# bearcove/loona

Hardware: AMD Instinct MI355X
Metric: Huffman header-literal decode GiB/s (device-resident) at 1/2/4/8 MI355X (higher is better)
Workload: dtype u8

## Files before the change

loona_amd/csrc/hpk_code.h:

```cpp
#pragma once
#include <stdint.h>

#define HPK_NSYM 257
#define HPK_EOS 256
#define HPK_LUT_BITS 12
#define HPK_LUT_SIZE (1u << HPK_LUT_BITS)
#define HPK_LO_RUNS 30
#define HPK_LO_SIZE (HPK_LO_RUNS * 32)

#define HPK_LIM5 0x50000000u
#define HPK_LIM6 0xB8000000u
#define HPK_LIM7 0xF8000000u
#define HPK_LIM8 0xFE000000u

static const uint8_t HPK_CODE_LEN[HPK_NSYM] = {
    13, 23, 28, 28, 28, 28, 28, 28, 28, 24, 30, 28, 28, 30, 28, 28,
    28, 28, 28, 28, 28, 28, 30, 28, 28, 28, 28, 28, 28, 28, 28, 28,
    6,  10, 10, 12, 13, 6,  8,  11, 10, 10, 8,  11, 8,  6,  6,  6,
    5,  5,  5,  6,  6,  6,  6,  6,  6,  6,  7,  8,  15, 6,  12, 10,
    13, 6,  7,  7,  7,  7,  7,  7,  7,  7,  7,  7,  7,  7,  7,  7,
    7,  7,  7,  7,  7,  7,  7,  7,  8,  7,  8,  13, 19, 13, 14, 6,
    15, 5,  6,  5,  6,  5,  6,  6,  6,  5,  7,  7,  6,  6,  6,  5,
    6,  7,  6,  5,  5,  6,  7,  7,  7,  7,  7,  15, 11, 14, 13, 28,
    20, 22, 20, 20, 22, 22, 22, 23, 22, 23, 23, 23, 23, 23, 24, 23,
    24, 24, 22, 23, 24, 23, 23, 23, 23, 21, 22, 23, 22, 23, 23, 24,
    22, 21, 20, 22, 22, 23, 23, 21, 23, 22, 22, 24, 21, 22, 23, 23,
    21, 21, 22, 21, 23, 22, 23, 23, 20, 22, 22, 22, 23, 22, 22, 23,
    26, 26, 20, 19, 22, 23, 22, 25, 26, 26, 26, 27, 27, 26, 24, 25,
    19, 21, 26, 27, 27, 26, 27, 24, 21, 21, 26, 26, 28, 27, 27, 27,
    20, 24, 20, 21, 22, 21, 21, 23, 22, 22, 25, 25, 24, 24, 26, 23,
    26, 27, 26, 26, 27, 27, 27, 27, 27, 28, 27, 27, 27, 27, 27, 26,
    30,
};

#define HPK_LUT2_NOTTWO 0x40000000u
#define HPK_LUT2_NONE 0x80000000u
#define HPK_LUT2_MISSING 15u
#define HPK_LUT2_CLAMP 14u
#define HPK_L2_LEN0(e) (((e) >> 8) & 15u)
#define HPK_L2_HELD(e) (((e) >> 12) & 15u)
#define HPK_L2_LEN01(e) (((e) >> 24) & 15u)
#define HPK_L2_CODES(e) (((e) >> 28) & 3u)
#define HPK_L2_TWO(e) (((e) >> 29) & 1u)

#define HPK_L3_HELD(e) (((e) >> 8) & 0xFFu)
#define HPK_L3_CODES(e) (((e) >> 24) & 3u)
#define HPK_L3_LEN0(e) (((e) >> 26) & 15u)
#define HPK_L3_NOTTWO 0x80000000u

struct hpk_tables {
    uint32_t code[HPK_NSYM];
    uint8_t len[HPK_NSYM];
    uint32_t lut[HPK_LUT_SIZE];
    uint32_t lut2[HPK_LUT_SIZE];
    uint32_t lut3[HPK_LUT_SIZE];
    uint16_t lo[HPK_LO_SIZE];
    uint8_t t8[256];
};

static inline int hpk_build_tables(hpk_tables* t) {
    uint16_t order[HPK_NSYM];
    int n = 0;
    for (int L = 1; L <= 30; ++L)
        for (int s = 0; s < HPK_NSYM; ++s)
            if (HPK_CODE_LEN[s] == L) order[n++] = (uint16_t)s;
    if (n != HPK_NSYM) return -1;
    uint64_t c = 0;
    int prev = HPK_CODE_LEN[order[0]];
    for (int i = 0; i < n; ++i) {
        int s = order[i], L = HPK_CODE_LEN[s];
        if (i) c = (c + 1) << (L - prev);
        prev = L;
        t->code[s] = (uint32_t)c;
        t->len[s] = (uint8_t)L;
    }
    if (c + 1 != (1ull << prev)) return -1;

    for (int k = 0; k < HPK_LO_RUNS; ++k)
        for (int t5 = 0; t5 < 32; ++t5) {
            uint64_t w = ((((1ull << k) - 1) << 6) | (uint64_t)t5) << (64 - (k + 6));
            uint16_t e = 0xFFFF;
            for (int s = 0; s < HPK_NSYM; ++s) {
                int L = t->len[s];
                if ((w >> (64 - L)) == t->code[s]) { e = (uint16_t)(s | (L << 9)); break; }
            }
            if (e == 0xFFFF) return -1;
            t->lo[k * 32 + t5] = e;
        }

    for (uint32_t v = 0; v < 256; ++v) {
        t->t8[v] = 0;
        const uint32_t w = v << 24;
        if (w >= HPK_LIM8) continue;
        const int L = 5 + (w >= HPK_LIM5) + (w >= HPK_LIM6) + (w >= HPK_LIM7);
        int found = -1;
        for (int s = 0; s < 256; ++s)
            if (t->len[s] <= 8 && (w >> (32 - t->len[s])) == t->code[s]) { found = s; break; }
        if (found < 0 || t->len[found] != L) return -1;
        t->t8[v] = (uint8_t)found;
    }

    for (uint32_t v = 0; v < HPK_LUT_SIZE; ++v) {
        uint32_t w = v << (32 - HPK_LUT_BITS);
        int s0 = -1, l0 = 0;
        for (int s = 0; s < 256; ++s) {
            int L = t->len[s];
            if (L <= HPK_LUT_BITS && (w >> (32 - L)) == t->code[s]) { s0 = s; l0 = L; break; }
        }
        if (s0 < 0) {
            t->lut[v] = 0;
            t->lut2[v] = 0xC0000000u | (HPK_LUT2_MISSING << 8) | (HPK_LUT2_MISSING << 24);
            continue;
        }
        uint32_t w1 = w << l0;
        int rem = HPK_LUT_BITS - l0, s1 = -1, l1 = 0;
        for (int s = 0; s < 256 && rem >= 5; ++s) {
            int L = t->len[s];
            if (L <= rem && (w1 >> (32 - L)) == t->code[s]) { s1 = s; l1 = L; break; }
        }
        uint32_t e = (uint32_t)s0 | ((uint32_t)l0 << 16);
        uint32_t e2 = (uint32_t)s0 | ((uint32_t)l0 << 8);
        if (s1 >= 0) {
            e |= ((uint32_t)s1 << 8) | ((uint32_t)(l0 + l1) << 21) | (2u << 26);
            e2 |= ((uint32_t)s1 << 16) | ((uint32_t)(l0 + l1) << 24) | ((uint32_t)(l0 + l1) << 12) | (2u << 28);
        } else {
            e |= ((uint32_t)l0 << 21) | (1u << 26);
            e2 |= (HPK_LUT2_MISSING << 24) | ((uint32_t)l0 << 12) | (1u << 28) | HPK_LUT2_NOTTWO;
        }
        t->lut[v] = e;
        t->lut2[v] = e2;
    }
    for (uint32_t v = 0; v < HPK_LUT_SIZE; ++v) {
        const uint32_t e2 = t->lut2[v], codes = HPK_L2_CODES(e2);
        t->lut3[v] = (e2 & 0xFFu) | (HPK_L2_HELD(e2) << 8) | (e2 & 0x00FF0000u) | (codes << 24) |
                     ((codes ? HPK_L2_LEN0(e2) : 15u) << 26) | (codes < 2 ? HPK_L3_NOTTWO : 0u);
    }
    return 0;
}
```

loona_amd/csrc/hpk_ctx.hip:

```cpp
#include <stdio.h>
#include <string.h>
#include <sys/mman.h>

#include <initializer_list>

#include "hpk_device.h"

#define HPK_VERSION "hpk 0.38 gfx950 decode v38 (every batch: wave fills, each wave with its own LDS window and image, longest-first queue, slot end offsets by DPP, nontemporal window loads stopping at the chunk's last byte, nontemporal write-back; chunks by guided self-scheduling from 4M literals, fixed 96-literal chunks below; fills and long-literal phase: body steps with no fit tests while >= 29 bits are left, then the wave fills' tails as four masked lookups with no fit test per code (checked steps only for a 13..28-bit code or a cut code in the tail) and the other kernels' checked tails (the long phase's at its refill points); long literals one lane each streaming from HBM after the fills, dense ranges listed longest-first; literals of >= 8 KiB by a whole workgroup in speculative pieces; compacted-output form: wave fills packed per workgroup from an LDS cursor into a bound layout made from the input offsets, each lane storing its two literals in unaligned 16-byte pieces; small-call mode: a persistent kernel behind a host-mapped doorbell); encode v5 (byte-balanced workgroup ranges, start map and DPP segmented scan, run accumulator, LDS image, live chunks only)"

static thread_local std::string t_last_error;

int hpk_set_err(const char* what, hipError_t e) {
    char buf[256];
    snprintf(buf, sizeof buf, "%s: %s", what, hipGetErrorString(e));
    t_last_error = buf;
    return HPK_E_DEVICE;
}

int hpk_set_err_msg(const char* what, int code) {
    t_last_error = what;
    return code;
}


extern "C" const char* hpk_version(void) { return HPK_VERSION; }

extern "C" const char* hpk_last_error(const hpk_ctx*) { return t_last_error.c_str(); }

extern "C" hpk_ctx* hpk_ctx_create(int device) {
    const hpk_tables* t = hpk_get_tables();
    if (!t) { hpk_set_err_msg("code table build failed", HPK_E_INVAL); return nullptr; }
    int ndev = 0;
    hipError_t e = hipGetDeviceCount(&ndev);
    if (e != hipSuccess || ndev <= 0) { hpk_set_err("hipGetDeviceCount", e); return nullptr; }
    if (device < 0 || device >= ndev) { hpk_set_err_msg("device index out of range", HPK_E_INVAL); return nullptr; }
    hpk_ctx* c = new hpk_ctx();
    c->device = device;
    auto fail = [&](const char* what, hipError_t err) {
        hpk_set_err(what, err);
        hpk_ctx_destroy(c);
        return (hpk_ctx*)nullptr;
    };
    if ((e = hipSetDevice(device)) != hipSuccess) return fail("hipSetDevice", e);
    hipDeviceProp_t prop;
    if ((e = hipGetDeviceProperties(&prop, device)) != hipSuccess) return fail("hipGetDeviceProperties", e);
    if (strncmp(prop.gcnArchName, "gfx950", 6) != 0) {
        hpk_set_err_msg("libhpk kernels are built for gfx950 only", HPK_E_NODEVICE);
        delete c;
        return nullptr;
    }
    c->num_cu = prop.multiProcessorCount;
    if ((e = hipStreamCreateWithFlags(&c->own, hipStreamNonBlocking)) != hipSuccess) return fail("hipStreamCreate", e);
    c->stream = c->own;
    if ((e = hipMalloc(&c->d_lut, sizeof(t->lut))) != hipSuccess) return fail("hipMalloc lut", e);
    if ((e = hipMemcpy(c->d_lut, t->lut, sizeof(t->lut), hipMemcpyHostToDevice)) != hipSuccess) return fail("upload lut", e);
    if ((e = hipMalloc(&c->d_lut2, sizeof(t->lut2))) != hipSuccess) return fail("hipMalloc lut2", e);
    if ((e = hipMemcpy(c->d_lut2, t->lut2, sizeof(t->lut2), hipMemcpyHostToDevice)) != hipSuccess)
        return fail("upload lut2", e);
    if ((e = hipMalloc(&c->d_lut3, sizeof(t->lut3))) != hipSuccess) return fail("hipMalloc lut3", e);
    if ((e = hipMemcpy(c->d_lut3, t->lut3, sizeof(t->lut3), hipMemcpyHostToDevice)) != hipSuccess)
        return fail("upload lut3", e);
    if ((e = hipMalloc(&c->d_lo, sizeof(t->lo))) != hipSuccess) return fail("hipMalloc lo", e);
    if ((e = hipMalloc(&c->d_t8, sizeof(t->t8))) != hipSuccess) return fail("hipMalloc t8", e);
    if ((e = hipMemcpy(c->d_t8, t->t8, sizeof(t->t8), hipMemcpyHostToDevice)) != hipSuccess) return fail("upload t8", e);
    if ((e = hipMalloc(&c->d_codes, 2 * 257 * sizeof(uint32_t))) != hipSuccess) return fail("hipMalloc codes", e);
    uint32_t packed[2 * 257];
    for (int s = 0; s < 257; ++s) {
        packed[s] = t->code[s];
        packed[257 + s] = t->len[s];
    }
    if ((e = hipMemcpy(c->d_lo, t->lo, sizeof(t->lo), hipMemcpyHostToDevice)) != hipSuccess) return fail("upload lo", e);
    if ((e = hipMemcpy(c->d_codes, packed, sizeof(packed), hipMemcpyHostToDevice)) != hipSuccess) return fail("upload codes", e);
    if ((e = hipHostMalloc((void**)&c->h_err, 64, hipHostMallocMapped | hipHostMallocCoherent)) != hipSuccess)
        return fail("hipHostMalloc err flag", e);
    *c->h_err = 0;
    if ((e = hipHostGetDevicePointer((void**)&c->d_err, c->h_err, 0)) != hipSuccess) return fail("err flag pointer", e);
    return c;
}

static int grow(void** p, size_t* cap, size_t need) {
    if (need <= *cap) return HPK_E_OK;
    size_t n = need + need / 4 + 4096;
    (void)hipFree(*p);
    *p = nullptr;
    *cap = 0;
    HIP_TRY(hipMalloc(p, n));
    *cap = n;
    return HPK_E_OK;
}

static int slot_acquire(hpk_ctx* c, hpk_slot** slot) {
    hpk_slot* s = nullptr;
    bool any = false;
    for (hpk_slot& k : c->slots) {
        if (k.used && k.stream == c->stream) s = &k;
        any |= k.used;
    }
    if (!s) {
        if (any && !c->slot_events) {
            c->slot_events = true;
            HIP_TRY(hipStreamSynchronize(c->own));
            for (hpk_slot& k : c->slots)
                if (k.stream == c->own) k.ev_set = false;
        }
        int j = 0;
        while (j < hpk_ctx::kSlots && c->slots[j].used) ++j;
        if (j == hpk_ctx::kSlots) {
            j = c->slot_next;
            c->slot_next = (j + 1) % hpk_ctx::kSlots;
            if (c->slots[j].ev_set) HIP_TRY(hipEventSynchronize(c->slots[j].ev));
        }
        s = &c->slots[j];
        s->stream = c->stream;
    }
    if (c->slot_events && !s->ev) HIP_TRY(hipEventCreateWithFlags(&s->ev, hipEventDisableTiming));
    *slot = s;
    return HPK_E_OK;
}

struct slot_need {
    DevBuf* buf;
    size_t bytes;
};
static int slot_reserve(hpk_ctx* c, hpk_slot* s, std::initializer_list<slot_need> needs) {
    bool small = false;
    for (const slot_need& nd : needs) small |= nd.buf->cap < nd.bytes;
    if (small) {
        if (s->ev_set)
            HIP_TRY(hipEventSynchronize(s->ev));
        else if (s->used)
            HIP_TRY(hipStreamSynchronize(c->own));
        for (const slot_need& nd : needs)
            if (int rc = grow(&nd.buf->p, &nd.buf->cap, nd.bytes)) return rc;
    }
    s->used = true;
    return HPK_E_OK;
}

static int slot_commit(hpk_ctx* c, hpk_slot* s) {
    if (!c->slot_events && c->stream == c->own) return HPK_E_OK;
    if (!s->ev) HIP_TRY(hipEventCreateWithFlags(&s->ev, hipEventDisableTiming));
    HIP_TRY(hipEventRecord(s->ev, c->stream));
    s->ev_set = true;
    return HPK_E_OK;
}

extern "C" void hpk_ctx_destroy(hpk_ctx* c) {
    if (!c) return;
    (void)hipSetDevice(c->device);
    (void)hpk_persist_stop(c);
    if (c->sm_stream) (void)hipStreamDestroy(c->sm_stream);
    if (c->h_sm) (void)hipHostFree(c->h_sm);
    (void)hipFree(c->d_sm_dev);
    (void)hipStreamSynchronize(c->stream);
    (void)hipFree(c->d_lut);
    (void)hipFree(c->d_lut2);
    (void)hipFree(c->d_lut3);
    (void)hipFree(c->d_lo);
    (void)hipFree(c->d_t8);
    (void)hipFree(c->d_codes);
    (void)hipFree(c->d_in);
    (void)hipFree(c->d_out);
    (void)hipFree(c->d_meta);
    (void)hipFree(c->d_st);
    if (c->h_err) (void)hipHostFree(c->h_err);
    if (c->h_pin) (void)hipHostFree(c->h_pin);
    for (hpk_slot& s : c->slots) {
        if (s.ev_set) (void)hipEventSynchronize(s.ev);
        for (DevBuf* b : {&s.long_list, &s.cp_bound, &s.cp_tmp, &s.cp_cursor, &s.pk_scratch, &s.pk_bound, &s.pk_tmp})
            (void)hipFree(b->p);
        if (s.ev) (void)hipEventDestroy(s.ev);
    }
    for (int j = 0; j < hpk_ctx::kMaxChunks; ++j) {
        if (c->ev_in[j]) (void)hipEventDestroy(c->ev_in[j]);
        if (c->ev_run[j]) (void)hipEventDestroy(c->ev_run[j]);
        if (c->ev_out[j]) (void)hipEventDestroy(c->ev_out[j]);
    }
    if (c->h2d) (void)hipStreamDestroy(c->h2d);
    if (c->d2h) (void)hipStreamDestroy(c->d2h);
    if (c->own) (void)hipStreamDestroy(c->own);
    delete c;
}

extern "C" int hpk_ctx_set_stream(hpk_ctx* c, void* s) {
    if (!c) return HPK_E_INVAL;
    if (s == HPK_STREAM_LEGACY)
        c->stream = (hipStream_t)0;
    else
        c->stream = s ? (hipStream_t)s : c->own;
    return HPK_E_OK;
}

extern "C" int hpk_host_register(void* ptr, size_t bytes) {
    if (!ptr || !bytes) return hpk_set_err_msg("null range", HPK_E_INVAL);
    HIP_TRY(hipHostRegister(ptr, bytes, hipHostRegisterDefault));
    return HPK_E_OK;
}

extern "C" int hpk_host_unregister(void* ptr) {
    if (!ptr) return hpk_set_err_msg("null pointer", HPK_E_INVAL);
    HIP_TRY(hipHostUnregister(ptr));
    return HPK_E_OK;
}

int hpk_ctx_pinned(hpk_ctx* c, size_t bytes, void** p) {
    if (bytes > c->h_pin_cap) {
        HIP_TRY(hipSetDevice(c->device));
        HIP_TRY(hipStreamSynchronize(c->stream));
        if (c->d2h) HIP_TRY(hipStreamSynchronize(c->d2h));
        if (c->h_pin) (void)hipHostFree(c->h_pin);
        c->h_pin = nullptr;
        c->h_pin_cap = 0;
        const size_t cap = bytes + bytes / 4 + (1u << 20);
        HIP_TRY(hipHostMalloc(&c->h_pin, cap, hipHostMallocDefault));
        c->h_pin_cap = cap;
    }
    *p = c->h_pin;
    return HPK_E_OK;
}

extern "C" int hpk_ctx_set_decode_kernel(hpk_ctx* c, int kind) {
    if (!c || kind < HPK_DECODE_AUTO || kind > HPK_DECODE_WAVE) return hpk_set_err_msg("bad decode kernel", HPK_E_INVAL);
    c->decode_kernel = kind;
    return HPK_E_OK;
}

extern "C" void* hpk_ctx_stream(hpk_ctx* c) { return c ? (void*)c->stream : nullptr; }

extern "C" int hpk_ctx_set_small_mode(hpk_ctx* c, uint32_t max_literals, int workgroups, uint32_t idle_ms) {
    if (!c) return HPK_E_INVAL;
    HIP_TRY(hipSetDevice(c->device));
    if (max_literals == 0) {
        const int rc = hpk_persist_stop(c);
        c->sm_max = 0;
        return rc;
    }
    if (workgroups < 1 || workgroups > 16 || workgroups >= c->num_cu || idle_ms < 1 || idle_ms > 10000 ||
        max_literals > (uint32_t)workgroups * 256u * 64u)
        return hpk_set_err_msg("small mode: 1-16 workgroups, 1-10000 ms idle, at most 64 literals per lane", HPK_E_INVAL);
    if (!c->h_sm) {
        HIP_TRY(hipStreamCreateWithFlags(&c->sm_stream, hipStreamNonBlocking));
        HIP_TRY(hipHostMalloc(&c->h_sm, 256, hipHostMallocMapped | hipHostMallocCoherent));
        memset(c->h_sm, 0, 256);
        HIP_TRY(hipHostGetDevicePointer(&c->d_sm, c->h_sm, 0));
        HIP_TRY(hipMalloc(&c->d_sm_dev, 128));
    }
    if (c->sm_launched && (workgroups != c->sm_wgs || idle_ms != c->sm_idle_ms))
        if (int rc = hpk_persist_stop(c)) return rc;
    c->sm_max = max_literals;
    c->sm_wgs = workgroups;
    c->sm_idle_ms = idle_ms;
    return c->sm_launched ? HPK_E_OK : hpk_persist_start(c);
}

extern "C" int hpk_ctx_sync(hpk_ctx* c) {
    if (!c) return HPK_E_INVAL;
    HIP_TRY(hipStreamSynchronize(c->stream));
    return HPK_E_OK;
}

static int check_offsets(const uint32_t* off, uint32_t n, size_t cap) {
    for (uint32_t i = 0; i < n; ++i)
        if (off[i + 1] < off[i]) return hpk_set_err_msg("offsets must be non-decreasing", HPK_E_INVAL);
    if (off[n] > cap || off[n] > HPK_MAX_OFFSET) return hpk_set_err_msg("offsets pass the blob's capacity", HPK_E_INVAL);
    return HPK_E_OK;
}

static int take_err(hpk_ctx* c) {
    if (!__atomic_exchange_n(c->h_err, 0u, __ATOMIC_ACQ_REL)) return HPK_E_OK;
    return hpk_set_err_msg("a batch had non-monotone offsets or offsets past a blob's capacity (HPK_BAD_OFFSETS)",
                           HPK_E_INVAL);
}

extern "C" int hpk_ctx_check(hpk_ctx* c) {
    if (!c) return HPK_E_INVAL;
    HIP_TRY(hipStreamSynchronize(c->stream));
    return take_err(c);
}

static int call_end(hpk_ctx* c, int flags) {
    if (flags & HPK_ASYNC) return HPK_E_OK;
    HIP_TRY(hipStreamSynchronize(c->stream));
    return take_err(c);
}

typedef int (*launch_fn)(hpk_ctx*, const hpk_batch&);

static int decode_region(hpk_ctx* c, const hpk_batch& b) {
    hpk_slot* s;
    int rc;
    if ((rc = slot_acquire(c, &s)) || (rc = slot_reserve(c, s, {{&s->long_list, 4 * (size_t)b.n}}))) return rc;
    if ((rc = hpk_launch_decode(c, b, s->long_list.as<uint32_t>()))) return rc;
    return slot_commit(c, s);
}

static uint32_t clamp_cap(size_t cap) { return cap > HPK_MAX_OFFSET ? HPK_MAX_OFFSET : (uint32_t)cap; }

static int queue_chunks(launch_fn fn, hpk_ctx* c, const uint8_t* in_blob, const uint32_t* in_off, uint8_t* out_blob,
                        const uint32_t* out_off, uint32_t* out_len, uint8_t* status, uint32_t n, size_t in_bytes,
                        size_t out_bytes, int chunks, const uint32_t* cut, uint32_t* d_in_off, uint32_t* d_out_off,
                        uint32_t* d_len);

static int host_begin(launch_fn fn, hpk_ctx* c, const uint8_t* in_blob, size_t in_cap, const uint32_t* in_off,
                      uint32_t n, uint8_t* out_blob, size_t out_cap, const uint32_t* out_off, uint32_t* out_len,
                      uint8_t* status, bool trusted, int* nchunks, uint32_t* cut) {
    *nchunks = 0;
    if (!trusted && (check_offsets(in_off, n, in_cap) || check_offsets(out_off, n, out_cap))) return HPK_E_INVAL;
    if (n == 0) return HPK_E_OK;
    const size_t in_bytes = in_off[n], out_bytes = out_off[n];
    if ((in_bytes && !in_blob) || (out_bytes && !out_blob)) return hpk_set_err_msg("null blob", HPK_E_INVAL);
    int rc;
    if ((rc = grow((void**)&c->d_in, &c->d_in_cap, in_bytes + 16))) return rc;
    if ((rc = grow((void**)&c->d_out, &c->d_out_cap, out_bytes + 16))) return rc;
    if ((rc = grow((void**)&c->d_meta, &c->d_meta_cap, (3 * (size_t)n + 2) * 4))) return rc;
    if ((rc = grow((void**)&c->d_st, &c->d_st_cap, n))) return rc;
    uint32_t* d_in_off = c->d_meta;
    uint32_t* d_out_off = c->d_meta + (n + 1);
    uint32_t* d_len = c->d_meta + 2 * ((size_t)n + 1);
    if (!c->h2d) {
        HIP_TRY(hipStreamCreateWithFlags(&c->h2d, hipStreamNonBlocking));
        HIP_TRY(hipStreamCreateWithFlags(&c->d2h, hipStreamNonBlocking));
        for (int j = 0; j < hpk_ctx::kMaxChunks; ++j) {
            HIP_TRY(hipEventCreateWithFlags(&c->ev_in[j], hipEventDisableTiming));
            HIP_TRY(hipEventCreateWithFlags(&c->ev_run[j], hipEventDisableTiming));
            HIP_TRY(hipEventCreateWithFlags(&c->ev_out[j], hipEventDisableTiming));
        }
    }
    const size_t kChunkBytes = (size_t)4 << 20;
    int chunks = (int)((in_bytes + out_bytes) / kChunkBytes);
    chunks = chunks < 1 ? 1 : (chunks > hpk_ctx::kMaxChunks ? hpk_ctx::kMaxChunks : chunks);
    if ((uint32_t)chunks > n) chunks = (int)n;
    cut[0] = 0;
    for (int j = 1; j < chunks; ++j) {
        const uint64_t target = (uint64_t)in_bytes * j / chunks;
        uint32_t lo = cut[j - 1], hi = n;
        while (lo < hi) {
            const uint32_t mid = lo + (hi - lo) / 2;
            if (in_off[mid + 1] < target) lo = mid + 1; else hi = mid;
        }
        cut[j] = lo;
    }
    cut[chunks] = n;
    auto drain = [&](int rc) {
        (void)hipStreamSynchronize(c->h2d);
        (void)hipStreamSynchronize(c->stream);
        (void)hipStreamSynchronize(c->d2h);
        return rc;
    };
    if (int e = queue_chunks(fn, c, in_blob, in_off, out_blob, out_off, out_len, status, n, in_bytes, out_bytes,
                             chunks, cut, d_in_off, d_out_off, d_len))
        return drain(e);
    *nchunks = chunks;
    return HPK_E_OK;
}

static int queue_chunks(launch_fn fn, hpk_ctx* c, const uint8_t* in_blob, const uint32_t* in_off, uint8_t* out_blob,
                        const uint32_t* out_off, uint32_t* out_len, uint8_t* status, uint32_t n, size_t in_bytes,
                        size_t out_bytes, int chunks, const uint32_t* cut, uint32_t* d_in_off, uint32_t* d_out_off,
                        uint32_t* d_len) {
    int rc;
    HIP_TRY(hipEventRecord(c->ev_run[0], c->stream));
    HIP_TRY(hipStreamWaitEvent(c->h2d, c->ev_run[0], 0));
    for (int j = 0; j < chunks; ++j) {
        const uint32_t a = cut[j], b = cut[j + 1];
        if (a < b) {
            const size_t ib = in_off[a], ie = in_off[b], ob = out_off[a], oe = out_off[b];
            if (ie > ib) HIP_TRY(hipMemcpyAsync(c->d_in + ib, in_blob + ib, ie - ib, hipMemcpyHostToDevice, c->h2d));
            HIP_TRY(hipMemcpyAsync(d_in_off + a, in_off + a, (b - a + 1) * 4ull, hipMemcpyHostToDevice, c->h2d));
            HIP_TRY(hipMemcpyAsync(d_out_off + a, out_off + a, (b - a + 1) * 4ull, hipMemcpyHostToDevice, c->h2d));
            HIP_TRY(hipEventRecord(c->ev_in[j], c->h2d));
            HIP_TRY(hipStreamWaitEvent(c->stream, c->ev_in[j], 0));
            const hpk_batch bt{c->d_in, (uint32_t)in_bytes, d_in_off + a, b - a, c->d_out, (uint32_t)out_bytes,
                               d_out_off + a, d_len + a, c->d_st + a};
            if ((rc = fn(c, bt))) return rc;
            HIP_TRY(hipEventRecord(c->ev_run[j], c->stream));
            HIP_TRY(hipStreamWaitEvent(c->d2h, c->ev_run[j], 0));
            if (oe > ob) HIP_TRY(hipMemcpyAsync(out_blob + ob, c->d_out + ob, oe - ob, hipMemcpyDeviceToHost, c->d2h));
            HIP_TRY(hipMemcpyAsync(out_len + a, d_len + a, (b - a) * 4ull, hipMemcpyDeviceToHost, c->d2h));
            HIP_TRY(hipMemcpyAsync(status + a, c->d_st + a, b - a, hipMemcpyDeviceToHost, c->d2h));
        }
        HIP_TRY(hipEventRecord(c->ev_out[j], c->d2h));
    }
    return HPK_E_OK;
}

static int host_end(hpk_ctx* c) {
    HIP_TRY(hipStreamSynchronize(c->d2h));
    return take_err(c);
}

static int run_batch(launch_fn fn, hpk_ctx* c, const uint8_t* in_blob, size_t in_cap, const uint32_t* in_off,
                     uint32_t n, uint8_t* out_blob, size_t out_cap, const uint32_t* out_off, uint32_t* out_len,
                     uint8_t* status, int flags) {
    if (!c || !in_off || !out_off || (n && (!out_len || !status))) return hpk_set_err_msg("null argument", HPK_E_INVAL);
    HIP_TRY(hipSetDevice(c->device));
    if (flags & HPK_PTR_DEVICE) {
        if (n == 0) return HPK_E_OK;
        if (!in_blob || !out_blob) return hpk_set_err_msg("null blob", HPK_E_INVAL);
        const hpk_batch b{in_blob, clamp_cap(in_cap), in_off, n, out_blob, clamp_cap(out_cap), out_off, out_len, status};
        if (fn == decode_region && !(flags & HPK_ASYNC) && c->sm_max) {
            bool handled = false;
            if (int rc = hpk_persist_call(c, b, &handled)) return rc;
            if (handled) return HPK_E_OK;
        }
        if (int rc = fn(c, b)) return rc;
        return call_end(c, flags);
    }
    int chunks;
    uint32_t cut[hpk_ctx::kMaxChunks + 1];
    if (int rc = host_begin(fn, c, in_blob, in_cap, in_off, n, out_blob, out_cap, out_off, out_len, status, false,
                            &chunks, cut))
        return rc;
    return chunks ? host_end(c) : HPK_E_OK;
}

int hpk_decode_host_begin(hpk_ctx* c, const uint8_t* in_blob, size_t in_cap, const uint32_t* in_off, uint32_t n,
                          uint8_t* out_blob, size_t out_cap, const uint32_t* out_off, uint32_t* out_len,
                          uint8_t* status, int* nchunks, uint32_t* cut) {
    HIP_TRY(hipSetDevice(c->device));
    return host_begin(decode_region, c, in_blob, in_cap, in_off, n, out_blob, out_cap, out_off, out_len, status,
                      true, nchunks, cut);
}

int hpk_host_chunk_wait(hpk_ctx* c, int j) {
    HIP_TRY(hipEventSynchronize(c->ev_out[j]));
    return HPK_E_OK;
}

int hpk_decode_host_end(hpk_ctx* c) { return host_end(c); }

int hpk_ctx_max_chunks() { return hpk_ctx::kMaxChunks; }

extern "C" int hpk_decode_batch(hpk_ctx* c, const uint8_t* in_blob, size_t in_cap, const uint32_t* in_off, uint32_t n,
                                uint8_t* out_blob, size_t out_cap, const uint32_t* out_off, uint32_t* out_len,
                                uint8_t* status, int flags) {
    return run_batch(decode_region, c, in_blob, in_cap, in_off, n, out_blob, out_cap, out_off, out_len, status,
                     flags);
}

static int check_call(const hpk_ctx* c, bool null_arg, int flags, uint32_t n, const char* what, const size_t* in_cap,
                      uint64_t* need) {
    auto inval = [&](const char* before, const char* after) {
        return hpk_set_err_msg((std::string(before) + what + after).c_str(), HPK_E_INVAL);
    };
    if (!c || null_arg) return hpk_set_err_msg("null argument", HPK_E_INVAL);
    if (!(flags & HPK_PTR_DEVICE)) return inval("the ", " takes device pointers only");
    if (n >= 0x7FFFFFFFu) return inval("too many literals for the ", "");
    if (in_cap) {
        *need = (uint64_t)hpk_decoded_bound(clamp_cap(*in_cap)) + 4ull * n;
        if (*need > HPK_MAX_OFFSET) return inval("the ", "'s output would pass 4 GiB");
    }
    return HPK_E_OK;
}

extern "C" int hpk_decode_batch_compact(hpk_ctx* c, const uint8_t* in_blob, size_t in_cap, const uint32_t* in_off,
                                        uint32_t n, uint8_t* out_blob, size_t out_cap, uint32_t* out_off,
                                        uint32_t* out_len, uint8_t* status, int flags) {
    uint64_t need;
    if (int rc = check_call(c, !in_off || !out_off || (n && (!out_len || !status)), flags, n, "compacted form", &in_cap,
                            &need))
        return rc;
    if (out_cap < need) return hpk_set_err_msg("out_cap below hpk_decoded_bound(in_cap) + 4 n", HPK_E_INVAL);
    HIP_TRY(hipSetDevice(c->device));
    if (n == 0) {
        HIP_TRY(hipMemsetAsync(out_off, 0, 4, c->stream));
        return call_end(c, flags);
    }
    if (!in_blob || !out_blob) return hpk_set_err_msg("null blob", HPK_E_INVAL);
    const bool wave = hpk_compact_wave(c, n);
    hpk_slot* s;
    int rc;
    if ((rc = slot_acquire(c, &s))) return rc;
    if (wave)
        rc = slot_reserve(c, s, {{&s->long_list, 4 * (size_t)n}});
    else
        rc = slot_reserve(c, s, {{&s->long_list, 4 * (size_t)n}, {&s->cp_bound, 4 * ((size_t)n + 1)},
                                 {&s->cp_tmp, hpk_bound_tmp_bytes(n)}, {&s->cp_cursor, 4}});
    if (rc) return rc;
    hpk_batch b{in_blob, clamp_cap(in_cap), in_off, n, out_blob, clamp_cap(out_cap), nullptr, out_len, status};
    uint32_t* cursor = nullptr;
    if (!wave) {
        b.out_off = s->cp_bound.as<uint32_t>();
        cursor = s->cp_cursor.as<uint32_t>();
        if ((rc = hpk_bound_scan(c, in_off, n, s->cp_bound.as<uint32_t>(), s->cp_tmp.p))) return rc;
        HIP_TRY(hipMemsetAsync(cursor, 0, 4, c->stream));
    }
    if ((rc = hpk_launch_decode_compact(c, b, out_off, s->long_list.as<uint32_t>(), cursor, wave))) return rc;
    if (!wave)
        HIP_TRY(hipMemcpyAsync(out_off + n, cursor, 4, hipMemcpyDeviceToDevice, c->stream));
    if ((rc = slot_commit(c, s))) return rc;
    return call_end(c, flags);
}

static int packed_end(hpk_ctx* c, const uint32_t* dst_off_n, size_t dst_cap, int flags) {
    if (flags & HPK_ASYNC) return HPK_E_OK;
    uint32_t total = 0;
    HIP_TRY(hipMemcpyAsync(&total, dst_off_n, 4, hipMemcpyDeviceToHost, c->stream));
    if (int rc = call_end(c, flags)) return rc;
    if ((size_t)total > dst_cap) return hpk_set_err_msg("the packed bytes pass the output capacity", HPK_E_NOSPACE);
    return HPK_E_OK;
}

extern "C" int hpk_decode_batch_packed(hpk_ctx* c, const uint8_t* in_blob, size_t in_cap, const uint32_t* in_off,
                                       uint32_t n, uint8_t* out_blob, size_t out_cap, uint32_t* out_off,
                                       uint32_t* out_len, uint8_t* status, int flags) {
    uint64_t need;
    if (int rc = check_call(c, !in_off || !out_off || (n && (!out_len || !status)), flags, n, "packed form", &in_cap, &need))
        return rc;
    if (n && (!in_blob || (!out_blob && out_cap))) return hpk_set_err_msg("null blob", HPK_E_INVAL);
    HIP_TRY(hipSetDevice(c->device));
    if (n == 0) {
        HIP_TRY(hipMemsetAsync(out_off, 0, 4, c->stream));
        return packed_end(c, out_off, out_cap, flags);
    }
    size_t tmp = hpk_bound_tmp_bytes(n);
    if (tmp < hpk_pack_tmp_bytes(n)) tmp = hpk_pack_tmp_bytes(n);
    hpk_slot* s;
    int rc;
    if ((rc = slot_acquire(c, &s)) ||
        (rc = slot_reserve(c, s, {{&s->long_list, 4 * (size_t)n}, {&s->pk_bound, 4 * ((size_t)n + 1)}, {&s->pk_tmp, tmp},
                                  {&s->pk_scratch, (size_t)need + 64}})))
        return rc;
    uint32_t* bound = s->pk_bound.as<uint32_t>();
    uint8_t* scratch = s->pk_scratch.as<uint8_t>();
    if ((rc = hpk_bound_scan(c, in_off, n, bound, s->pk_tmp.p))) return rc;
    const hpk_batch b{in_blob, clamp_cap(in_cap), in_off, n, scratch, (uint32_t)need, bound, out_len, status};
    if ((rc = hpk_launch_decode(c, b, s->long_list.as<uint32_t>()))) return rc;
    if ((rc = hpk_pack_launch(c, scratch, (uint32_t)need, bound, out_len, n, out_blob, clamp_cap(out_cap), out_off,
                              s->pk_tmp.p, need)))
        return rc;
    if ((rc = slot_commit(c, s))) return rc;
    return packed_end(c, out_off + n, out_cap, flags);
}

extern "C" int hpk_pack_batch(hpk_ctx* c, const uint8_t* src_blob, size_t src_cap, const uint32_t* src_off,
                              const uint32_t* src_len, uint32_t n, uint8_t* dst_blob, size_t dst_cap, uint32_t* dst_off,
                              int flags) {
    if (int rc = check_call(c, !dst_off || (n && (!src_off || !src_len)), flags, n, "pack", nullptr, nullptr)) return rc;
    if (n && ((!src_blob && src_cap) || (!dst_blob && dst_cap))) return hpk_set_err_msg("null blob", HPK_E_INVAL);
    HIP_TRY(hipSetDevice(c->device));
    hpk_slot* s;
    int rc;
    if ((rc = slot_acquire(c, &s)) || (rc = slot_reserve(c, s, {{&s->pk_tmp, hpk_pack_tmp_bytes(n)}}))) return rc;
    if ((rc = hpk_pack_launch(c, src_blob, clamp_cap(src_cap), src_off, src_len, n, dst_blob, clamp_cap(dst_cap), dst_off,
                              s->pk_tmp.p, HPK_MAX_OFFSET)))
        return rc;
    if ((rc = slot_commit(c, s))) return rc;
    return packed_end(c, dst_off + n, dst_cap, flags);
}

extern "C" int hpk_encode_batch(hpk_ctx* c, const uint8_t* in_blob, size_t in_cap, const uint32_t* in_off, uint32_t n,
                                uint8_t* out_blob, size_t out_cap, const uint32_t* out_off, uint32_t* out_len,
                                uint8_t* status, int flags) {
    return run_batch(hpk_launch_encode, c, in_blob, in_cap, in_off, n, out_blob, out_cap, out_off, out_len, status,
                     flags);
}

struct hpk_arena {
    void* base;
    size_t len;
    int pinned;
};

extern "C" hpk_arena* hpk_arena_create(size_t num_bufs, size_t buf_size, int pin) {
    if (!num_bufs || !buf_size || num_bufs > ((size_t)1 << 40) / buf_size) {
        hpk_set_err_msg("bad arena size", HPK_E_INVAL);
        return nullptr;
    }
    const size_t len = num_bufs * buf_size;
    void* p = mmap(nullptr, len, PROT_READ | PROT_WRITE, MAP_PRIVATE | MAP_ANONYMOUS, -1, 0);
    if (p == MAP_FAILED) {
        hpk_set_err_msg("mmap failed", HPK_E_INVAL);
        return nullptr;
    }
    hpk_arena* a = new hpk_arena{p, len, 0};
    if (pin) {
        const hipError_t e = hipHostRegister(p, len, hipHostRegisterDefault);
        if (e != hipSuccess) {
            hpk_set_err("hipHostRegister arena", e);
            munmap(p, len);
            delete a;
            return nullptr;
        }
        a->pinned = 1;
    }
    return a;
}

extern "C" void* hpk_arena_base(const hpk_arena* a) { return a ? a->base : nullptr; }
extern "C" size_t hpk_arena_len(const hpk_arena* a) { return a ? a->len : 0; }

extern "C" void hpk_arena_destroy(hpk_arena* a) {
    if (!a) return;
    if (a->pinned) (void)hipHostUnregister(a->base);
    munmap(a->base, a->len);
    delete a;
}
```

loona_amd/csrc/hpk_decode.hip:

```cpp
#include <stdlib.h>

#include <chrono>

#include "hpk_fill.h"
#include "hpk_wave.h"
#include "hpk_persist.h"

using namespace hpkdec;

constexpr int kWaves = 16, kW = 40960, kO = 79104, kQ = 2048, kRefillN = 2;
#ifndef HPK_LONG_MIN
#define HPK_LONG_MIN 64
#endif
#ifndef HPK_LONG_BIG
#define HPK_LONG_BIG 1024
#endif
using Geo = Geo12<kWaves, kW, kO, kQ>;
constexpr int kWaveWin = 3072, kWaveImg = 5888;
#ifndef HPK_WAVE_MIN
#define HPK_WAVE_MIN 0u
#endif
#ifndef HPK_WAVE_GUIDED
#define HPK_WAVE_GUIDED 1
#endif
#ifndef HPK_WAVE_RANK
#define HPK_WAVE_RANK 0
#endif
#ifndef HPK_WAVE_CHUNK
#define HPK_WAVE_CHUNK 224u
#endif
#define WAVE_KERNEL(m) hpk_decode_wave<m, kWaveWin, kWaveImg, HPK_WAVE_CHUNK, HPK_WAVE_GUIDED, HPK_WAVE_RANK>
#ifndef HPK_WAVE_GUIDED_MIN
#define HPK_WAVE_GUIDED_MIN 4000000u
#endif
#ifndef HPK_WAVE_SMALL_CHUNK
#define HPK_WAVE_SMALL_CHUNK 96u
#endif
#define WAVE_KERNEL_SMALL(m) hpk_decode_wave<m, kWaveWin, kWaveImg, HPK_WAVE_SMALL_CHUNK, 2, HPK_WAVE_RANK>
#define DEC_KERNEL(m) hpk_decode12<m, kWaves, kW, kO, kQ, kRefillN>

#ifdef HPK_DIAG
static int g_debug_mode = -1;
static unsigned long long* g_dbg = nullptr;
static size_t g_dbg_n = 0;

static int dbg_buffer(hpk_ctx* c, DecodeArgs& a, size_t need, bool zero) {
    if (need > g_dbg_n) {
        (void)hipFree(g_dbg);
        HIP_TRY(hipMalloc(&g_dbg, need * 8));
        g_dbg_n = need;
    }
    if (zero) HIP_TRY(hipMemsetAsync(g_dbg, 0, need * 8, c->stream));
    a.dbg = g_dbg;
    return HPK_E_OK;
}

extern "C" int hpk_debug_check(unsigned long long* host8) {
    return hipMemcpyFromSymbol(host8, HIP_SYMBOL(g_chk), 8 * sizeof(unsigned long long)) == hipSuccess ? 0 : -1;
}

extern "C" int hpk_debug_stamps(unsigned long long* host, size_t cap_entries) {
    if (!g_dbg) return 0;
    size_t n = g_dbg_n < cap_entries ? g_dbg_n : cap_entries;
    if (hipMemcpy(host, g_dbg, n * 8, hipMemcpyDeviceToHost) != hipSuccess) return -1;
    return (int)n;
}
#endif

static void decode_args(hpk_ctx* c, const hpk_batch& b, DecodeArgs& a) {
    const auto in = split16(b.in_blob);
    const auto out = split16(b.out_blob);
    a.in_base = in.base;
    a.in_mis = in.mis;
    a.in_off = b.in_off;
    a.n = b.n;
    a.out_base = out.base;
    a.out_mis = out.mis;
    a.out_off = b.out_off;
    a.out_len = b.out_len;
    a.status = b.status;
    a.t8 = c->d_t8;
    a.lo = c->d_lo;
    a.lut = c->d_lut;
    a.lut2 = c->d_lut2;
    a.lut3 = c->d_lut3;
    a.dbg = nullptr;
    a.in_cap = b.in_cap;
    a.out_cap = b.out_cap;
    a.err = c->d_err;
    a.lit_out = b.out_off;
    a.co_off = nullptr;
    a.cursor = nullptr;
}

static uint32_t decode_blocks(hpk_ctx* c, const hpk_batch& b) {
    uint64_t blocks = ((uint64_t)b.n + 63) / 64;
    if (blocks < ((uint64_t)b.in_cap + 32767) / 32768) blocks = ((uint64_t)b.in_cap + 32767) / 32768;
    if (blocks > (uint64_t)b.n) blocks = (uint64_t)b.n;
    const uint64_t cus = (uint64_t)c->num_cu - (c->sm_launched && c->sm_max ? (uint64_t)c->sm_wgs : 0u);
    if (blocks > cus) blocks = cus;
    if (blocks < 1) blocks = 1;
    return (uint32_t)blocks;
}

constexpr int kPersistThreads = 256;

static int persist_launch(hpk_ctx* c, uint32_t base) {
    auto* h = static_cast<PersistCtl*>(c->h_sm);
    if (c->sm_launched) HIP_TRY(hipStreamSynchronize(c->sm_stream));
    __atomic_store_n(&h->stop, 0u, __ATOMIC_RELAXED);
    __atomic_store_n(&h->done, base, __ATOMIC_RELAXED);
    __atomic_store_n(&h->declined, 0u, __ATOMIC_RELAXED);
    __atomic_store_n(&h->alive, 1u, __ATOMIC_RELEASE);
    const uint32_t init[4] = {0u, base, 0u, 0u};
    HIP_TRY(hipMemcpyAsync(c->d_sm_dev, init, sizeof init, hipMemcpyHostToDevice, c->sm_stream));
    PersistArgs a{static_cast<PersistCtl*>(c->d_sm), c->d_sm_dev, c->d_lut3, c->d_lo, base, c->sm_idle_ms * 100000u};
    hipLaunchKernelGGL(hpk_persist<kPersistThreads>, dim3((uint32_t)c->sm_wgs), dim3(kPersistThreads), 0, c->sm_stream, a);
    HIP_TRY(hipGetLastError());
    c->sm_launched = true;
    return HPK_E_OK;
}

int hpk_persist_start(hpk_ctx* c) { return persist_launch(c, c->sm_req); }

extern "C" uint64_t hpk_test_small_calls(const hpk_ctx* c) { return c ? c->sm_calls : 0u; }

extern "C" int hpk_test_small_stamps(const hpk_ctx* c, uint32_t* out10) {
    if (!c || !c->h_sm || !out10) return HPK_E_INVAL;
    const auto* h = static_cast<const PersistCtl*>(c->h_sm);
    for (int k = 0; k < 6; ++k) out10[k] = __atomic_load_n(&h->ts[k], __ATOMIC_ACQUIRE);
    for (int k = 0; k < 4; ++k) out10[6 + k] = __atomic_load_n(&h->tl[k], __ATOMIC_ACQUIRE);
    return HPK_E_OK;
}

int hpk_persist_stop(hpk_ctx* c) {
    if (!c->sm_launched) return HPK_E_OK;
    auto* h = static_cast<PersistCtl*>(c->h_sm);
    __atomic_store_n(&h->stop, 1u, __ATOMIC_RELEASE);
    HIP_TRY(hipStreamSynchronize(c->sm_stream));
    c->sm_launched = false;
    return HPK_E_OK;
}

int hpk_persist_call(hpk_ctx* c, const hpk_batch& b, bool* handled) {
    *handled = false;
    if (!c->sm_max || b.n > c->sm_max || b.n == 0) return HPK_E_OK;
    if (hipStreamQuery(c->stream) != hipSuccess) HIP_TRY(hipStreamSynchronize(c->stream));
    auto* h = static_cast<PersistCtl*>(c->h_sm);
    if (!c->sm_launched || __atomic_load_n(&h->alive, __ATOMIC_ACQUIRE) == 0u)
        if (int rc = persist_launch(c, c->sm_req)) return rc;
    const auto in = split16(b.in_blob);
    const auto out = split16(b.out_blob);
    h->in_base = in.base;
    h->out_base = out.base;
    h->in_off = b.in_off;
    h->out_off = b.out_off;
    h->out_len = b.out_len;
    h->status = b.status;
    h->n = b.n;
    h->in_mis = in.mis;
    h->out_mis = out.mis;
    h->in_cap = b.in_cap;
    h->out_cap = b.out_cap;
    const uint32_t k = ++c->sm_req;
    __atomic_store_n(&h->req, k, __ATOMIC_RELEASE);
    const auto t0 = std::chrono::steady_clock::now();
    for (uint32_t spins = 0; __atomic_load_n(&h->done, __ATOMIC_ACQUIRE) != k; ++spins) {
        if (__atomic_load_n(&h->alive, __ATOMIC_ACQUIRE) == 0u) {
            if (int rc = persist_launch(c, k - 1u)) return rc;
        }
        __builtin_ia32_pause();
        if ((spins & 4095u) == 4095u && std::chrono::steady_clock::now() - t0 > std::chrono::seconds(10))
            return hpk_set_err_msg("small-call mode: the persistent kernel did not answer", HPK_E_DEVICE);
    }
    *handled = __atomic_load_n(&h->declined, __ATOMIC_ACQUIRE) == 0u;
    c->sm_calls += *handled ? 1u : 0u;
    return HPK_E_OK;
}

bool hpk_compact_wave(const hpk_ctx* c, uint32_t n) {
    return c->decode_kernel == HPK_DECODE_WAVE || (c->decode_kernel == HPK_DECODE_AUTO && n >= HPK_WAVE_MIN);
}

int hpk_launch_decode_compact(hpk_ctx* c, const hpk_batch& b, uint32_t* co_off, uint32_t* long_list, uint32_t* cursor,
                              bool wave) {
    DecodeArgs a;
    decode_args(c, b, a);
    a.lit_out = co_off;
    a.co_off = co_off;
    a.cursor = cursor;
    a.long_list = long_list;
    a.long_min = HPK_LONG_MIN;
    a.long_big = HPK_LONG_BIG;
    if (wave) {
        a.cursor = nullptr;
        hipLaunchKernelGGL((hpk_decode_wave<0, kWaveWin, kWaveImg, HPK_WAVE_CHUNK, HPK_WAVE_GUIDED, HPK_WAVE_RANK, true>),
                           dim3(decode_blocks(c, b)), dim3(Geo::kBlock), 0, c->stream, a);
    } else {
        hipLaunchKernelGGL((hpk_decode12<0, kWaves, kW, kO, kQ, kRefillN, true>), dim3(decode_blocks(c, b)),
                           dim3(Geo::kBlock), 0, c->stream, a);
    }
    HIP_TRY(hipGetLastError());
    return HPK_E_OK;
}

int hpk_launch_decode(hpk_ctx* c, const hpk_batch& b, uint32_t* long_list) {
    DecodeArgs a;
    decode_args(c, b, a);
    a.long_list = long_list;
    a.long_min = HPK_LONG_MIN;
    a.long_big = HPK_LONG_BIG;
#ifdef HPK_DIAG
    if (const char* lm = getenv("HPK_LONG_MIN")) a.long_min = (uint32_t)atoi(lm);
    if (const char* lb = getenv("HPK_LONG_BIG")) a.long_big = (uint32_t)atoi(lb);
#endif
    const uint32_t blocks = decode_blocks(c, b);
    const dim3 grid(blocks), block(Geo::kBlock);
    bool wave = c->decode_kernel == HPK_DECODE_WAVE || (c->decode_kernel == HPK_DECODE_AUTO && b.n >= HPK_WAVE_MIN);
#ifdef HPK_DIAG
    if (const char* wk = getenv("HPK_DECODE_KERNEL")) wave = wk[0] == 'w';
    if (g_debug_mode < 0) {
        const char* dm = getenv("HPK_DEBUG_MODE");
        g_debug_mode = dm ? atoi(dm) : 0;
    }
    static const int wave_var = getenv("HPK_WAVE_VARIANT") ? atoi(getenv("HPK_WAVE_VARIANT")) : -1;
    if (wave && wave_var >= 0 && g_debug_mode == 0) {
        switch (wave_var) {
            case 0: hipLaunchKernelGGL((hpk_decode_wave<0, kWaveWin, kWaveImg, 224u, false, 0>), grid, block, 0, c->stream, a); break;
            case 1: hipLaunchKernelGGL((hpk_decode_wave<0, kWaveWin, kWaveImg, 224u, false, 1>), grid, block, 0, c->stream, a); break;
            case 2: hipLaunchKernelGGL((hpk_decode_wave<0, kWaveWin, kWaveImg, 224u, false, 2>), grid, block, 0, c->stream, a); break;
            case 3: hipLaunchKernelGGL((hpk_decode_wave<0, kWaveWin, kWaveImg, 224u, true, 0>), grid, block, 0, c->stream, a); break;
            case 4: hipLaunchKernelGGL((hpk_decode_wave<0, kWaveWin, kWaveImg, 224u, true, 1>), grid, block, 0, c->stream, a); break;
            case 5: hipLaunchKernelGGL((hpk_decode_wave<0, kWaveWin, kWaveImg, 224u, true, 2>), grid, block, 0, c->stream, a); break;
            default: hipLaunchKernelGGL((WAVE_KERNEL(0)), grid, block, 0, c->stream, a); break;
        }
        HIP_TRY(hipGetLastError());
        return HPK_E_OK;
    }
    if (g_debug_mode == 3 || g_debug_mode == 5) {
        const size_t waves = g_debug_mode == 3 ? kWaves : HPK_LONG_WAVES;
        if (int rc = dbg_buffer(c, a, (size_t)blocks * waves * 16, g_debug_mode == 5)) return rc;
    }
#define WAVE_MODE(m)                                                                  \
    case m:                                                                           \
        if (b.n < HPK_WAVE_GUIDED_MIN)                                                \
            hipLaunchKernelGGL(WAVE_KERNEL_SMALL(m), grid, block, 0, c->stream, a);   \
        else                                                                          \
            hipLaunchKernelGGL(WAVE_KERNEL(m), grid, block, 0, c->stream, a);         \
        break;
#define FILL_MODE(m) \
    case m: hipLaunchKernelGGL(DEC_KERNEL(m), grid, block, 0, c->stream, a); break;
    if (wave) {
        switch (g_debug_mode) {
            WAVE_MODE(1) WAVE_MODE(2) WAVE_MODE(3) WAVE_MODE(5) WAVE_MODE(6) WAVE_MODE(8) WAVE_MODE(9) WAVE_MODE(10)
            default: WAVE_MODE(0)
        }
    } else {
        switch (g_debug_mode) {
            FILL_MODE(1) FILL_MODE(2) FILL_MODE(3) FILL_MODE(4) FILL_MODE(5)
            default: FILL_MODE(0)
        }
    }
#else
    if (wave && b.n < HPK_WAVE_GUIDED_MIN)
        hipLaunchKernelGGL(WAVE_KERNEL_SMALL(0), grid, block, 0, c->stream, a);
    else if (wave)
        hipLaunchKernelGGL(WAVE_KERNEL(0), grid, block, 0, c->stream, a);
    else
        hipLaunchKernelGGL(DEC_KERNEL(0), grid, block, 0, c->stream, a);
#endif
    HIP_TRY(hipGetLastError());
    return HPK_E_OK;
}
```

loona_amd/csrc/hpk_decode_kernel.h:

```cpp
#pragma once
#include <stdint.h>

#include "hpk_device.h"
#include "hpk_walk.h"

namespace hpkdec {

constexpr int kT8Bytes = 256;
constexpr int kLoBytes = HPK_LO_SIZE * 2;
constexpr int kTabBytes = ((kT8Bytes + kLoBytes + 15) / 16) * 16;

struct DecodeArgs {
    const uint8_t* in_base;
    uint32_t in_mis;
    const uint32_t* in_off;
    uint32_t n;
    uint8_t* out_base;
    uint32_t out_mis;
    const uint32_t* out_off;
    uint32_t* out_len;
    uint8_t* status;
    const uint8_t* t8;
    const uint16_t* lo;
    const uint32_t* lut;
    const uint32_t* lut2;
    const uint32_t* lut3;
    unsigned long long* dbg;
    uint32_t in_cap, out_cap;
    uint32_t* err;
    uint32_t* long_list;
    uint32_t long_min, long_big;
    const uint32_t* lit_out;
    uint32_t* co_off;
    uint32_t* cursor;
};

constexpr uint32_t kHugeMax = 16;

typedef uint32_t u32u __attribute__((aligned(1)));
typedef uint32_t u32x4u __attribute__((ext_vector_type(4), aligned(1)));

constexpr uint32_t kListed = 0xFFFFFFFFu;

constexpr uint32_t kQ7Byte = 0x80000000u;

__device__ __forceinline__ uint32_t lpt_bucket(uint32_t nbytes) {
    const uint32_t b = nbytes < 96u ? (nbytes >> 1) : min(63u, 48u + ((nbytes - 96u) >> 7));
    return 63u - b;
}

__device__ __forceinline__ void lds_barrier() { asm volatile("s_waitcnt lgkmcnt(0)\n\ts_barrier" ::: "memory"); }

}
```

loona_amd/csrc/hpk_device.h:

```cpp
#pragma once
#include <hip/hip_runtime.h>
#include <stdint.h>

#include <string>

#include "../../include/hpk.h"
#include "hpk_code.h"
#include "hpk_internal.h"

template <class T>
struct hpk_split16 {
    T* base;
    uint32_t mis;
};
template <class T>
inline hpk_split16<T> split16(T* p) {
    const uintptr_t u = (uintptr_t)p;
    return {(T*)(u & ~(uintptr_t)15), (uint32_t)(u & 15)};
}

struct DevBuf {
    void* p = nullptr;
    size_t cap = 0;
    template <class T>
    T* as() const { return static_cast<T*>(p); }
};

struct hpk_slot {
    hipStream_t stream = nullptr;
    bool used = false;
    hipEvent_t ev = nullptr;
    bool ev_set = false;
    DevBuf long_list;
    DevBuf cp_bound, cp_tmp, cp_cursor;
    DevBuf pk_scratch, pk_bound, pk_tmp;
};

struct hpk_ctx {
    int device = 0;
    int num_cu = 256;
    int decode_kernel = HPK_DECODE_AUTO;
    hipStream_t own = nullptr;
    hipStream_t stream = nullptr;
    uint32_t* d_lut = nullptr;
    uint32_t* d_lut2 = nullptr;
    uint32_t* d_lut3 = nullptr;
    uint16_t* d_lo = nullptr;
    uint8_t* d_t8 = nullptr;
    uint32_t* d_codes = nullptr;
    uint8_t* d_in = nullptr;
    size_t d_in_cap = 0;
    uint8_t* d_out = nullptr;
    size_t d_out_cap = 0;
    uint32_t* d_meta = nullptr;
    size_t d_meta_cap = 0;
    uint8_t* d_st = nullptr;
    size_t d_st_cap = 0;
    void* h_pin = nullptr;
    size_t h_pin_cap = 0;
    static constexpr int kMaxChunks = 8;
    hipStream_t h2d = nullptr;
    hipStream_t d2h = nullptr;
    hipEvent_t ev_in[kMaxChunks] = {};
    hipEvent_t ev_run[kMaxChunks] = {};
    hipEvent_t ev_out[kMaxChunks] = {};
    uint32_t* h_err = nullptr;
    uint32_t* d_err = nullptr;
    static constexpr int kSlots = 8;
    hpk_slot slots[kSlots];
    int slot_next = 0;
    bool slot_events = false;
    uint32_t sm_max = 0;
    int sm_wgs = 0;
    uint32_t sm_idle_ms = 0;
    hipStream_t sm_stream = nullptr;
    void* h_sm = nullptr;
    void* d_sm = nullptr;
    uint32_t* d_sm_dev = nullptr;
    uint32_t sm_req = 0;
    bool sm_launched = false;
    uint64_t sm_calls = 0;
};

int hpk_persist_call(hpk_ctx* c, const struct hpk_batch& b, bool* handled);
int hpk_persist_start(hpk_ctx* c);
int hpk_persist_stop(hpk_ctx* c);

struct hpk_batch {
    const uint8_t* in_blob;
    uint32_t in_cap;
    const uint32_t* in_off;
    uint32_t n;
    uint8_t* out_blob;
    uint32_t out_cap;
    const uint32_t* out_off;
    uint32_t* out_len;
    uint8_t* status;
};

int hpk_set_err(const char* what, hipError_t e);
int hpk_set_err_msg(const char* what, int code);

#define HIP_TRY(call)                                            \
    do {                                                         \
        hipError_t _e = (call);                                  \
        if (_e != hipSuccess) return hpk_set_err(#call, _e);     \
    } while (0)

int hpk_launch_decode(hpk_ctx* c, const hpk_batch& b, uint32_t* long_list);
bool hpk_compact_wave(const hpk_ctx* c, uint32_t n);
int hpk_launch_decode_compact(hpk_ctx* c, const hpk_batch& b, uint32_t* co_off, uint32_t* long_list, uint32_t* cursor,
                              bool wave);
int hpk_launch_encode(hpk_ctx* c, const hpk_batch& b);
size_t hpk_bound_tmp_bytes(uint32_t n);
int hpk_bound_scan(hpk_ctx* c, const uint32_t* in_off, uint32_t n, uint32_t* out, void* tmp);
size_t hpk_pack_tmp_bytes(uint32_t n);
int hpk_pack_launch(hpk_ctx* c, const uint8_t* src_blob, uint32_t src_cap, const uint32_t* src_off, const uint32_t* src_len,
                    uint32_t n, uint8_t* dst_blob, uint32_t dst_cap, uint32_t* dst_off, void* tmp, uint64_t total_bound);

__device__ __forceinline__ uint32_t hpk_bswap32(uint32_t x) { return __builtin_bswap32(x); }
```

loona_amd/csrc/hpk_huge_piece.h:

```cpp
#pragma once
#include "hpk_walk.h"

namespace hpkdec {

#ifndef HPK_HUGE_MIN
#define HPK_HUGE_MIN 8192u
#endif
constexpr uint32_t kHugePieceMin = 64;
constexpr uint32_t kHugeTerm = 0x100u;
constexpr uint32_t kHugeNone = 0xFFFFFFFFu;
constexpr uint32_t kHugeLimit = 1u << 28;

struct HugeWalk {
    uint64_t win;
    uint32_t nb;
    uint32_t qi;
    uint32_t pos;
    uint4 c0, c1;
};

__device__ __forceinline__ uint32_t huge_sel(const uint4& c, uint32_t j) {
    const uint32_t sh = (j & 1u) * 32u;
    const uint32_t lo = (uint32_t)((((uint64_t)c.y << 32) | c.x) >> sh);
    const uint32_t hi = (uint32_t)((((uint64_t)c.w << 32) | c.z) >> sh);
    return (j & 2u) ? hi : lo;
}

template <class Ld>
__device__ __forceinline__ void huge_begin(HugeWalk& W, const Ld& ld16, uint32_t lbyte, uint32_t pos) {
    const uint32_t b = lbyte + (pos >> 3);
    const uint32_t qd = b >> 2;
    const uint32_t sk = (b & 3u) * 8u + (pos & 7u);
    W.c0 = ld16(qd >> 2);
    W.c1 = ld16((qd >> 2) + 1u);
    W.win = ((uint64_t)__builtin_bswap32(huge_sel(W.c0, qd & 3u)) << 32) << sk;
    W.nb = 32u - sk;
    W.qi = qd + 1u;
    W.pos = pos;
    if ((W.qi & 3u) == 0u) {
        W.c0 = W.c1;
        W.c1 = ld16((W.qi >> 2) + 1u);
    }
}

template <int kTab, class Ld>
__device__ __forceinline__ void huge_peek(HugeWalk& W, const Ld& ld16, const uint32_t* __restrict__ lut,
                                          const uint16_t* __restrict__ lo, uint32_t& sym, uint32_t& len, bool& eos,
                                          uint32_t& sym1, uint32_t& held) {
    if (W.nb <= 32u) {
        W.win |= (uint64_t)__builtin_bswap32(huge_sel(W.c0, W.qi & 3u)) << (32u - W.nb);
        W.nb += 32u;
        W.qi += 1u;
        if ((W.qi & 3u) == 0u) {
            W.c0 = W.c1;
            W.c1 = ld16((W.qi >> 2) + 1u);
        }
    }
    const uint32_t w = (uint32_t)(W.win >> 32);
    const uint32_t e = lut[w >> (32 - HPK_LUT_BITS)];
    const uint32_t l0 = kTab == 3 ? HPK_L3_LEN0(e) : HPK_L2_LEN0(e);
    if (l0 <= (uint32_t)HPK_LUT_BITS) {
        sym = e & 0xFFu;
        len = l0;
        eos = false;
        const uint32_t codes = kTab == 3 ? HPK_L3_CODES(e) : HPK_L2_CODES(e);
        held = codes == 2u ? (kTab == 3 ? HPK_L3_HELD(e) : HPK_L2_HELD(e)) : 0u;
        sym1 = (e >> 16) & 0xFFu;
    } else {
        lo_decode(w, lo, sym, len, eos);
        held = 0;
        sym1 = 0;
    }
}

__device__ __forceinline__ void huge_adv(HugeWalk& W, uint32_t len) {
    W.win <<= len;
    W.nb -= len;
    W.pos += len;
}

template <int kTab, class Ld>
__device__ __forceinline__ uint32_t huge_count(HugeWalk& W, const Ld& ld16, const uint32_t* __restrict__ lut,
                                               const uint16_t* __restrict__ lo, uint32_t nbits, uint32_t nx, bool last,
                                               uint32_t& c) {
    c = 0;
    for (;;) {
        if (!last && W.pos >= nx) return 0u;
        uint32_t sym, len, sym1, held;
        bool eos;
        huge_peek<kTab>(W, ld16, lut, lo, sym, len, eos, sym1, held);
        const uint32_t rem = nbits - W.pos;
        if (held != 0u && held <= rem && (last || W.pos + len < nx)) {
            huge_adv(W, held);
            c += 2u;
            continue;
        }
        if (len > rem) return kHugeTerm | residual_status(rem, (uint32_t)(W.win >> 32));
        if (eos) return kHugeTerm | HPK_EOS_IN_STRING;
        huge_adv(W, len);
        c += 1u;
    }
}

__device__ __forceinline__ void huge_geometry(uint32_t nbytes, uint32_t lanes, uint32_t& P, uint32_t& PB, uint32_t& OV) {
    P = min(lanes, (nbytes + kHugePieceMin - 1u) / kHugePieceMin);
    PB = (nbytes + P - 1u) / P;
    P = (nbytes + PB - 1u) / PB;
    OV = PB >= 512u ? 512u : 256u;
}

template <int kTab, class Ld>
__device__ __forceinline__ void huge_pass1(const Ld& ld16, const uint32_t* __restrict__ lut, const uint16_t* __restrict__ lo,
                                           uint32_t lbyte, uint32_t nbytes, uint32_t k, uint32_t P, uint32_t PB,
                                           uint32_t OV, uint32_t& S, uint32_t& E, uint32_t& c, uint32_t& fl) {
    const uint32_t nbits = nbytes * 8u, st = k * PB * 8u;
    const bool last = k + 1u == P;
    const uint32_t nx = last ? nbits : (k + 1u) * PB * 8u;
    HugeWalk W;
    huge_begin(W, ld16, lbyte, k == 0u ? 0u : (st > OV ? st - OV : 0u));
    c = 0;
    fl = 0;
    while (W.pos < st) {
        uint32_t sym, len, sym1, held;
        bool eos;
        huge_peek<kTab>(W, ld16, lut, lo, sym, len, eos, sym1, held);
        if (held != 0u && held <= nbits - W.pos && W.pos + len < st) {
            huge_adv(W, held);
            continue;
        }
        if (len > nbits - W.pos || eos) {
            S = E = kHugeNone;
            return;
        }
        huge_adv(W, len);
    }
    S = W.pos;
    fl = huge_count<kTab>(W, ld16, lut, lo, nbits, nx, last, c);
    E = W.pos;
}

template <int kTab, class Ld>
__device__ __forceinline__ void huge_refix(const Ld& ld16, const uint32_t* __restrict__ lut, const uint16_t* __restrict__ lo,
                                           uint32_t lbyte, uint32_t nbytes, uint32_t k, uint32_t P, uint32_t PB,
                                           uint32_t from, uint32_t& S, uint32_t& E, uint32_t& c, uint32_t& fl) {
    const uint32_t nbits = nbytes * 8u;
    const bool last = k + 1u == P;
    const uint32_t nx = last ? nbits : (k + 1u) * PB * 8u;
    HugeWalk W;
    huge_begin(W, ld16, lbyte, from);
    S = from;
    fl = huge_count<kTab>(W, ld16, lut, lo, nbits, nx, last, c);
    E = W.pos;
}

template <int kTab, class Ld, class St8, class St1>
__device__ __forceinline__ void huge_pass2(const Ld& ld16, const uint32_t* __restrict__ lut, const uint16_t* __restrict__ lo,
                                           uint32_t lbyte, uint32_t S, uint32_t c, uint32_t ob, const St8& st8,
                                           const St1& st1) {
    HugeWalk W;
    huge_begin(W, ld16, lbyte, S);
    uint64_t acc = 0;
    uint32_t p = ob;
    auto emit = [&](uint32_t sym) {
        acc |= (uint64_t)sym << (8u * (p & 7u));
        if ((p & 7u) == 7u) {
            const uint32_t g = p - 7u;
            if (g >= ob) {
                st8(g, acc);
            } else {
                for (uint32_t x = ob; x <= p; ++x) st1(x, (uint8_t)(acc >> (8u * (x & 7u))));
            }
            acc = 0;
        }
        p += 1u;
    };
    for (uint32_t j = 0; j < c;) {
        uint32_t sym, len, sym1, held;
        bool eos;
        huge_peek<kTab>(W, ld16, lut, lo, sym, len, eos, sym1, held);
        emit(sym);
        if (held != 0u && j + 2u <= c) {
            emit(sym1);
            huge_adv(W, held);
            j += 2u;
        } else {
            huge_adv(W, len);
            j += 1u;
        }
    }
    for (uint32_t x = max(ob, p & ~7u); x < p; ++x) st1(x, (uint8_t)(acc >> (8u * (x & 7u))));
}

}
```

loona_amd/csrc/hpk_long.h:

```cpp
#pragma once
#include "hpk_decode_kernel.h"

namespace hpkdec {

typedef uint32_t u32x4 __attribute__((ext_vector_type(4)));

__device__ __forceinline__ __amdgpu_buffer_rsrc_t buf_rsrc(const void* p, uint32_t bytes) {
    return __builtin_amdgcn_make_buffer_rsrc(const_cast<void*>(p), 0, (int)bytes, 0x00020000);
}

__device__ __forceinline__ void store_part(__amdgpu_buffer_rsrc_t r, uint32_t gb, uint32_t lo, uint32_t hi,
                                           const uint32_t (&v)[4], const uint32_t (&b)[16]) {
#pragma unroll
    for (uint32_t d = 0; d < 4u; ++d) {
        if (lo <= 4u * d && 4u * d + 4u <= hi) {
            __builtin_amdgcn_raw_buffer_store_b32(v[d], r, gb, 4 * d, 0);
        } else {
#pragma unroll
            for (uint32_t e = 0; e < 4u; ++e)
                if (4u * d + e >= lo && 4u * d + e < hi)
                    __builtin_amdgcn_raw_buffer_store_b8((uint8_t)b[4u * d + e], r, gb, 4 * d + e, 0);
        }
    }
}

__device__ __forceinline__ uint32_t lpt_class_of(uint32_t nb);

__device__ __forceinline__ void pin(uint32_t x) { asm volatile("" ::"v"(x)); }

#ifndef HPK_LONG_WAVES
#define HPK_LONG_WAVES 8
#endif
#ifndef HPK_LONG_U
#define HPK_LONG_U 8
#endif
#ifndef HPK_LONG_CLAIM
#define HPK_LONG_CLAIM 64
#endif
#ifndef HPK_LONG_RING
#define HPK_LONG_RING 32
#endif

#ifndef HPK_LONG_TAILPT
#define HPK_LONG_TAILPT 1
#endif

#ifndef HPK_LONG_CH
#define HPK_LONG_CH 3
#endif

#ifndef HPK_LONG_OS
#define HPK_LONG_OS 80
#endif

#ifndef HPK_LONG_BODY
#define HPK_LONG_BODY 1
#endif

__device__ __forceinline__ uint32_t lpt_class_of(uint32_t nb) { return 31u - min(nb >> 7, 31u); }

template <int kBlock, int kU, int kRing, int kDiag, int kBlockAll, int kOSz = HPK_LONG_OS, int kClaim = 64,
          int kTab = 2,
          bool kCompact = false,
          int kCh = HPK_LONG_CH>
__device__ __forceinline__ void long_phase(const DecodeArgs& a, uint32_t ba, uint32_t bb, uint32_t c1, uint32_t c2,
                                           uint32_t* s_claim, uint32_t* s_ring, uint8_t* s_out, uint4* s_q,
                                           const uint32_t* s_lut, const uint16_t* s_lo) {
    constexpr uint32_t kChunk = kClaim;
    constexpr uint32_t kQ = kChunk;
    static_assert(kClaim == 32 || kClaim == 64, "claim size");
    constexpr uint32_t kOS = kOSz;
    static_assert(15 + 5 * kU + 3 + (HPK_LONG_TAILPT ? 6 : 0) < (int)kOS, "output buffer");
    static_assert((kRing & (kRing - 1)) == 0 && kRing >= 16 && 4 * kCh + 8 <= kRing, "input ring: a power of two >= 16 dwords");
    static_assert(kBlock % 64 == 0 && kBlock <= kBlockAll, "decoding waves");
    const uint32_t tid = threadIdx.x, lane = tid & 63u, wv = tid >> 6;
    const uint32_t total = c1 + c2;
    if (total == 0) return;
    if (tid >= (uint32_t)kBlock) return;
    uint4 (*sq)[kQ] = reinterpret_cast<uint4 (*)[kQ]>(s_q);
    const uint32_t in_end = min(a.in_off[a.n], a.in_cap) + a.in_mis;
    const __amdgpu_buffer_rsrc_t r_in = buf_rsrc(a.in_base, (in_end + 15u) & ~15u);
    const __amdgpu_buffer_rsrc_t r_out = buf_rsrc(a.out_base, a.out_cap + a.out_mis);
    const __amdgpu_buffer_rsrc_t r_len = buf_rsrc(a.out_len, min(a.n, 0x3FFFFFFFu) * 4u);
    const __amdgpu_buffer_rsrc_t r_st = buf_rsrc(a.status, a.n);
    uint32_t* ring = s_ring + tid;
    uint8_t* const obuf = s_out + tid * kOS;
    bool more = true;
    uint32_t qh = 0, qt = 0;
    bool act = false, live = false, pend = false, done = false;
    uint32_t idx = 0, X = 0, Eb = 0, d0 = 0, d1 = 0, d2 = 0, st = HPK_OK, q0 = 0, span = 0, h = 0;
    uint32_t o0 = 0, ob = 0, fl = 0, lb = 0;
    u32x4 P[kCh] = {};
    unsigned long long dg[12] = {};
    const unsigned long long dt0 = kDiag ? __builtin_amdgcn_s_memtime() : 0;
    for (;;) {
        unsigned long long dtp = kDiag ? __builtin_amdgcn_s_memtime() : 0;
        if (kDiag) dg[1] += 1;
        if (pend) {
            if (kDiag) asm volatile("s_waitcnt vmcnt(0)" ::: "memory");
            const uint32_t b = h & (kRing - 1u);
#pragma unroll
            for (int c = 0; c < kCh; ++c) {
                ring[((b + 4 * c + 0) & (kRing - 1u)) * kBlock] = __builtin_bswap32(P[c].x);
                ring[((b + 4 * c + 1) & (kRing - 1u)) * kBlock] = __builtin_bswap32(P[c].y);
                ring[((b + 4 * c + 2) & (kRing - 1u)) * kBlock] = __builtin_bswap32(P[c].z);
                ring[((b + 4 * c + 3) & (kRing - 1u)) * kBlock] = __builtin_bswap32(P[c].w);
            }
            h += 4u * kCh;
            pend = false;
        }
        if (kDiag) {
            const unsigned long long t = __builtin_amdgcn_s_memtime();
            dg[11] += t - dtp;
        }
        if (act && !live && (h != 0 || span == 0)) {
            const uint32_t j = X >> 5;
            d0 = ring[((j - 1u) & (kRing - 1u)) * kBlock];
            d1 = ring[j * kBlock];
            d2 = ring[(j + 1u) * kBlock];
            live = true;
        }
        if (HPK_LONG_TAILPT) {
            for (;;) {
                const bool tl = act && live && !done && Eb - X < kBodyMin && h * 4u >= span;
                if (!__any(tl)) break;
                if (tl) {
                    const uint32_t j0 = X >> 5;
                    const uint32_t d3 = ring[((j0 + 2u) & (kRing - 1u)) * kBlock];
                    const uint32_t w = __builtin_amdgcn_alignbit(d0, d1, ~X);
                    const uint32_t rem = Eb - X;
                    const uint32_t e1 = s_lut[w >> (32 - HPK_LUT_BITS)];
                    bool a1, a2;
                    const uint32_t u1 = lut12<kTab>(e1, rem, a1, a2);
                    bool park = !a1 & (rem > (uint32_t)HPK_LUT_BITS);
                    const bool cont = a1 & (a2 | lut_nottwo<kTab>(e1));
                    const uint32_t rem2 = rem - u1;
                    const uint32_t e2 = s_lut[(w << u1) >> (32 - HPK_LUT_BITS)];
                    bool b1, b2;
                    const uint32_t v2 = lut12<kTab>(e2, rem2, b1, b2);
                    park |= cont & !b1 & (rem2 > (uint32_t)HPK_LUT_BITS);
                    b1 &= cont;
                    b2 &= cont;
                    const uint32_t g1 = (uint32_t)a1 + (uint32_t)a2, g2 = (uint32_t)b1 + (uint32_t)b2;
                    uint8_t* const p = obuf + (ob - lb);
                    p[0] = (uint8_t)e1;
                    p[1] = (uint8_t)(e1 >> 16);
                    p[g1] = (uint8_t)e2;
                    p[g1 + 1] = (uint8_t)(e2 >> 16);
                    ob += g1 + g2;
                    const uint32_t xn = X + u1 + (cont ? v2 : 0u);
                    const bool cross = (xn ^ X) > 31u;
                    d0 = cross ? d1 : d0;
                    d1 = cross ? d2 : d1;
                    d2 = cross ? d3 : d2;
                    X = xn;
                    bool prog = a1 | park;
                    const bool mo = park | (b1 & (b2 | lut_nottwo<kTab>(e2)));
                    if (park) {
                        const uint32_t wp = __builtin_amdgcn_alignbit(d0, d1, ~X);
                        uint32_t sy, len;
                        bool eos;
                        lo_decode(wp, s_lo, sy, len, eos);
                        if (len > Eb - X) {
                            st = HPK_PADDING_TOO_LARGE;
                            prog = false;
                        } else if (eos) {
                            st = HPK_EOS_IN_STRING;
                            prog = false;
                        } else {
                            obuf[ob - lb] = (uint8_t)sy;
                            ob += 1u;
                            const uint32_t xp = X + len;
                            const uint32_t j = xp >> 5;
                            d0 = ring[((j - 1u) & (kRing - 1u)) * kBlock];
                            d1 = ring[(j & (kRing - 1u)) * kBlock];
                            d2 = ring[((j + 1u) & (kRing - 1u)) * kBlock];
                            X = xp;
                        }
                    }
                    done = !prog || !mo;
                }
            }
        }
        u32x4 gv[4];
        uint32_t hv[4], hb[16], tv[4], tb[16], lv = 0, sv = 0;
        uint32_t ha = 0, ga = 0, ta = 0, ia = 0, ja = 0;
        {
            const uint32_t gb = fl & ~15u;
            ha = gb;
            if (act && fl != gb && gb + 16u <= ob) {
                const uint32_t* s = reinterpret_cast<const uint32_t*>(obuf);
#pragma unroll
                for (int e = 0; e < 4; ++e) hv[e] = s[e];
#pragma unroll
                for (int e = 0; e < 16; ++e) hb[e] = hv[e >> 2] >> (8 * (e & 3));
                store_part(r_out, gb, fl - gb, 16u, hv, hb);
                fl = gb + 16u;
            }
        }
        {
            ga = fl;
#pragma unroll
            for (int k = 0; k < 4; ++k) {
                const uint32_t* s = reinterpret_cast<const uint32_t*>(obuf + min((fl - lb) + 16u * k, kOS - 16u));
                gv[k] = u32x4{s[0], s[1], s[2], s[3]};
            }
            uint32_t ng = 0;
#pragma unroll
            for (int k = 0; k < 4; ++k) {
                if (act && ga + 16u * (k + 1) <= ob) {
                    __builtin_amdgcn_raw_buffer_store_b128(gv[k], r_out, ga, 16 * k, 0);
                    ng = k + 1;
                }
            }
            fl += 16u * ng;
            if (act && fl != lb && (fl & 15u) == 0) {
                const uint4 v = *reinterpret_cast<const uint4*>(obuf + (fl - lb));
                *reinterpret_cast<uint4*>(obuf) = v;
                lb = fl;
            }
        }
        if (done) {
            if (st == HPK_OK) st = residual_status(Eb - X, __builtin_amdgcn_alignbit(d0, d1, ~X));
            if (ob > fl) {
                const uint32_t gb = fl & ~15u;
                ta = gb;
                const uint32_t* s = reinterpret_cast<const uint32_t*>(obuf);
#pragma unroll
                for (int e = 0; e < 4; ++e) tv[e] = s[e];
#pragma unroll
                for (int e = 0; e < 16; ++e) tb[e] = tv[e >> 2] >> (8 * (e & 3));
                store_part(r_out, gb, fl - gb, ob - gb, tv, tb);
            }
            lv = ob - o0;
            sv = st;
            ia = idx * 4u;
            ja = idx;
            __builtin_amdgcn_raw_buffer_store_b32(lv, r_len, ia, 0, 0);
            __builtin_amdgcn_raw_buffer_store_b8((uint8_t)sv, r_st, ja, 0, 0);
            act = false;
            live = false;
            done = false;
        }
        if (kDiag) {
            const unsigned long long t = __builtin_amdgcn_s_memtime();
            dg[7] += t - dtp;
            dtp = t;
        }
#pragma unroll 1
        for (int claims = 0;; ++claims) {
            const bool want = !act;
            if (!__any(want)) break;
            const uint64_t wm = __ballot(want);
            const uint32_t rank = __builtin_amdgcn_mbcnt_hi((uint32_t)(wm >> 32), __builtin_amdgcn_mbcnt_lo((uint32_t)wm, 0u));
            if (want && qh + rank < qt) {
                const uint4 te = sq[wv][(qh + rank) % kQ];
                idx = te.x;
                act = true;
                live = false;
                const uint32_t p0 = te.y + a.in_mis, p1 = te.z + a.in_mis;
                q0 = p0 >> 4;
                span = p1 - (q0 << 4);
                X = (p0 & 15u) * 8u + 31u;
                Eb = X + (p1 - p0) * 8u;
                h = 0;
                st = HPK_OK;
                o0 = te.w + a.out_mis;
                ob = o0;
                fl = o0;
                lb = o0 & ~15u;
            }
            const uint32_t need = (uint32_t)__popcll(wm);
            const bool enough = need <= qt - qh;
            qh += min(need, qt - qh);
            if (enough || !more || claims == 2) break;
            uint32_t rr = 0;
            if (lane == 0) rr = atomicAdd(s_claim, kChunk);
            const uint32_t r = (uint32_t)__builtin_amdgcn_readlane((int)rr, 0);
            if (r >= total) {
                more = false;
                break;
            }
            const uint32_t e = r + lane;
            const bool ok = lane < kChunk && e < total;
            const uint32_t lpos = ok ? (e < c1 ? ba + e : bb - 1u - (e - c1)) : ba;
            const uint32_t i0 = a.long_list[lpos];
            const uint32_t i = ok ? i0 : 0u;
            uint4 li;
            if (kCompact) {
                li = make_uint4(i, a.in_off[i], a.in_off[i + 1], 0u);
                const uint32_t bd = ok ? ((li.z - li.y) * 8u) / 5u : 0u;
                uint32_t x = bd;
#pragma unroll
                for (int d = 1; d < 64; d <<= 1) {
                    const uint32_t y = __shfl_up(x, d);
                    if (lane >= (uint32_t)d) x += y;
                }
                uint32_t cb = 0;
                if (lane == 63u) cb = atomicAdd(a.cursor, x);
                li.w = (uint32_t)__builtin_amdgcn_readlane((int)cb, 63) + x - bd;
                if (ok) a.co_off[i] = li.w;
            } else {
                li = make_uint4(i, a.in_off[i], a.in_off[i + 1], a.lit_out[i]);
            }
            const uint64_t lm = __ballot(ok);
            const uint32_t lr = __builtin_amdgcn_mbcnt_hi((uint32_t)(lm >> 32), __builtin_amdgcn_mbcnt_lo((uint32_t)lm, 0u));
            if (ok) sq[wv][(qt + lr) % kQ] = li;
            qt += (uint32_t)__popcll(lm);
        }
        if (kDiag) {
            const unsigned long long t = __builtin_amdgcn_s_memtime();
            dg[5] += t - dtp;
            dtp = t;
        }
        if (!__any(act)) break;
        if (act && h * 4u < span && h + 4u * kCh + 1u <= kRing + (X >> 5)) {
#pragma unroll
            for (int c = 0; c < kCh; ++c)
                P[c] = __builtin_amdgcn_raw_buffer_load_b128(r_in, (q0 + (h >> 2)) * 16u + 16u * c, 0, 0);
            pend = true;
        }
        const uint32_t x5 = X >> 5;
        const uint32_t budget = !(act && live) ? 0u
                                : h * 4u >= span ? (uint32_t)kU
                                : x5 + 4u <= h ? min((uint32_t)kU, ((h - x5 - 4u) >> 1) + 1u) : 0u;
        for (int s = 0; s < kU; ++s) {
            const bool go = (uint32_t)s < budget && !done && (!HPK_LONG_TAILPT || Eb - X >= kBodyMin);
            if (kDiag) {
                dg[2] += (unsigned long long)__popcll(__ballot(go));
                dg[3] += (unsigned long long)__popcll(__ballot(act && live && !done && !go));
                dg[4] += (unsigned long long)__popcll(__ballot(!act));
                dg[9] += (unsigned long long)__popcll(__ballot(act && !live));
                dg[10] += (unsigned long long)__popcll(__ballot(act && live && done));
            }
            if (!go) continue;
            const uint32_t j0 = X >> 5;
            const uint32_t d3 = ring[((j0 + 2u) & (kRing - 1u)) * kBlock];
            const uint32_t w = __builtin_amdgcn_alignbit(d0, d1, ~X);
            const uint32_t rem = Eb - X;
            uint32_t e1, e2, u1, u2, g1, g2;
            bool park, prog;
            if (HPK_LONG_TAILPT || (HPK_LONG_BODY && rem >= kBodyMin)) {
                e1 = s_lut[w >> (32 - HPK_LUT_BITS)];
                u1 = kTab == 3 ? HPK_L3_HELD(e1) : HPK_L2_HELD(e1);
                e2 = s_lut[(w << u1) >> (32 - HPK_LUT_BITS)];
                u2 = kTab == 3 ? HPK_L3_HELD(e2) : HPK_L2_HELD(e2);
                g1 = kTab == 3 ? HPK_L3_CODES(e1) : HPK_L2_CODES(e1);
                g2 = kTab == 3 ? HPK_L3_CODES(e2) : HPK_L2_CODES(e2);
                park = u2 == 0u;
                prog = true;
            } else {
                e1 = s_lut[w >> (32 - HPK_LUT_BITS)];
                bool a1, a2;
                u1 = lut12<kTab>(e1, rem, a1, a2);
                park = !a1 & (rem > (uint32_t)HPK_LUT_BITS);
                const bool cont = a1 & (a2 | lut_nottwo<kTab>(e1));
                const uint32_t w2 = w << u1;
                const uint32_t rem2 = rem - u1;
                e2 = s_lut[w2 >> (32 - HPK_LUT_BITS)];
                bool b1, b2;
                const uint32_t v2 = lut12<kTab>(e2, rem2, b1, b2);
                park |= cont & !b1 & (rem2 > (uint32_t)HPK_LUT_BITS);
                b1 &= cont;
                b2 &= cont;
                g1 = (uint32_t)a1 + (uint32_t)a2;
                g2 = (uint32_t)b1 + (uint32_t)b2;
                u2 = cont ? v2 : 0u;
                prog = a1 | park;
            }
            {
                uint8_t* const p = obuf + (ob - lb);
                p[0] = (uint8_t)e1;
                p[1] = (uint8_t)(e1 >> 16);
                p[g1] = (uint8_t)e2;
                p[g1 + 1] = (uint8_t)(e2 >> 16);
                ob += g1 + g2;
            }
            const uint32_t xn = X + u1 + u2;
            const bool cross = (xn ^ X) > 31u;
            d0 = cross ? d1 : d0;
            d1 = cross ? d2 : d1;
            d2 = cross ? d3 : d2;
            X = xn;
            if (park) {
                const uint32_t wp = __builtin_amdgcn_alignbit(d0, d1, ~X);
                uint32_t sy, len;
                bool eos;
                lo_decode(wp, s_lo, sy, len, eos);
                if (len > Eb - X) {
                    st = HPK_PADDING_TOO_LARGE;
                    prog = false;
                } else if (eos) {
                    st = HPK_EOS_IN_STRING;
                    prog = false;
                } else {
                    obuf[ob - lb] = (uint8_t)sy;
                    ob += 1u;
                    const uint32_t xp = X + len;
                    const uint32_t j = xp >> 5;
                    d0 = ring[((j - 1u) & (kRing - 1u)) * kBlock];
                    d1 = ring[(j & (kRing - 1u)) * kBlock];
                    d2 = ring[((j + 1u) & (kRing - 1u)) * kBlock];
                    X = xp;
                }
            }
            done = !prog;
        }
        if (kDiag) dg[6] += __builtin_amdgcn_s_memtime() - dtp;
#pragma unroll
        for (int k = 0; k < 4; ++k) {
            pin(gv[k].x);
            pin(gv[k].y);
            pin(gv[k].z);
            pin(gv[k].w);
            pin(hv[k]);
            pin(tv[k]);
        }
#pragma unroll
        for (int e = 0; e < 16; ++e) {
            pin(hb[e]);
            pin(tb[e]);
        }
        pin(lv);
        pin(sv);
        pin(ha);
        pin(ga);
        pin(ta);
        pin(ia);
        pin(ja);
    }
    if (kDiag) {
        dg[0] = __builtin_amdgcn_s_memtime() - dt0;
        const uint32_t gw = blockIdx.x * (uint32_t)(kBlock / 64) + wv;
        if (lane < 12) {
            unsigned long long v = 0;
#pragma unroll
            for (int i = 0; i < 12; ++i) v = lane == (uint32_t)i ? dg[i] : v;
            a.dbg[gw * 16u + lane] = v;
        }
    }
}

}
```

loona_amd/csrc/hpk_walk.h:

```cpp
#pragma once
#include <stdint.h>

#include "../../include/hpk.h"
#include "hpk_code.h"

namespace hpkdec {

enum StoreMode { kDword = 0, kNoStore = 1, kChecked = 3, kPred = 4 };

#ifdef __HIPCC__
__device__ unsigned long long g_chk[8];
__device__ __forceinline__ void chk_report(uint32_t code, uint32_t a0, uint32_t a1, uint32_t a2) {
    if (atomicCAS(&g_chk[0], 0ull, (unsigned long long)code) == 0ull) {
        g_chk[1] = a0;
        g_chk[2] = a1;
        g_chk[3] = a2;
        g_chk[4] = blockIdx.x;
        g_chk[5] = threadIdx.x;
    }
}
#else
inline void chk_report(uint32_t, uint32_t, uint32_t, uint32_t) {}
#endif

__device__ __forceinline__ void put8(uint8_t* __restrict__ out8, uint32_t pos, uint32_t v, uint32_t oend, int kStore) {
    if (kStore == kChecked) {
        if (pos < oend)
            out8[pos] = (uint8_t)v;
        else
            chk_report(1, pos, oend, 0);
    } else if (kStore == kDword || kStore == kPred) {
        out8[pos] = (uint8_t)v;
    } else {
        asm volatile("" ::"v"(v));
    }
}

__device__ __forceinline__ uint32_t win_at(const uint32_t* __restrict__ win32, uint32_t p) {
    const uint32_t x = p + 31u;
    const uint32_t* q = win32 + (x >> 5);
    return __builtin_amdgcn_alignbit(q[-1], q[0], ~x);
}

template <int kTab = 2>
__device__ __forceinline__ uint32_t lut12(uint32_t e, uint32_t rem, bool& ok1, bool& ok2) {
    const uint32_t rc = min(rem, HPK_LUT2_CLAMP);
    if (kTab == 3) {
        const uint32_t l1 = HPK_L3_LEN0(e), t1 = HPK_L3_HELD(e);
        ok1 = l1 <= rc;
        ok2 = (t1 <= rc) & (e < HPK_L3_NOTTWO);
        return ok2 ? t1 : (ok1 ? l1 : 0u);
    }
    const uint32_t l1 = HPK_L2_LEN0(e), t1 = HPK_L2_LEN01(e);
    ok1 = l1 <= rc;
    ok2 = t1 <= rc;
    return ok2 ? t1 : (ok1 ? l1 : 0u);
}
template <int kTab>
__device__ __forceinline__ bool lut_nottwo(uint32_t e) {
    return kTab == 3 ? e >= HPK_L3_NOTTWO : e >= HPK_LUT2_NOTTWO;
}
template <int kTab>
__device__ __forceinline__ uint32_t lut_sym1(uint32_t e) {
    return e >> 16;
}

__device__ __forceinline__ uint32_t residual_status(uint32_t rem, uint32_t w) {
    if (rem == 0) return HPK_OK;
    if (rem > 7) return HPK_PADDING_TOO_LARGE;
    return (w | (0xFFFFFFFFu >> rem)) != 0xFFFFFFFFu ? HPK_INVALID_PADDING : HPK_OK;
}

__device__ __forceinline__ void lo_decode(uint32_t w, const uint16_t* __restrict__ lo, uint32_t& sym,
                                          uint32_t& len, bool& eos) {
    const uint32_t kk = __clz(~w);
    const uint32_t e = lo[min(kk, (uint32_t)HPK_LO_RUNS - 1) * 32 + ((w << ((kk + 1) & 31)) >> 27)];
    eos = kk >= HPK_LO_RUNS || (e & 0x1FFu) == HPK_EOS;
    sym = e & 0xFFu;
    len = eos ? 30u : (e >> 9);
}


struct Lit12 {
    uint32_t X;
    uint32_t Eb;
    uint32_t d0, d1, d2;
    uint32_t o;
    uint32_t o0;
    uint32_t oend;
    uint32_t st;
    uint32_t idx;
    bool prog;
    bool more;
    bool act;
};

__device__ __forceinline__ void lit12_load(Lit12& L, const uint32_t* __restrict__ win32) {
    const uint32_t* p = win32 + (L.X >> 5);
    L.d0 = p[-1];
    L.d1 = p[0];
    L.d2 = p[1];
}

template <int kStore, bool kP1, int kTab, bool kMore>
__device__ __forceinline__ bool lit12_step_main(Lit12& L, const uint32_t* __restrict__ win32,
                                                const uint32_t* __restrict__ lut, uint8_t* __restrict__ out8,
                                                uint32_t dmy) {
    const uint32_t d3 = win32[(L.X >> 5) + 2];
    const uint32_t w = __builtin_amdgcn_alignbit(L.d0, L.d1, ~L.X);
    const uint32_t rem = L.Eb - L.X;
    const uint32_t e1 = lut[w >> (32 - HPK_LUT_BITS)];
    bool a1, a2;
    const uint32_t u1 = lut12<kTab>(e1, rem, a1, a2);
    uint32_t use = u1;
    bool park = !a1 & (rem > (uint32_t)HPK_LUT_BITS);
    bool more2 = false;
    if (kStore == kPred) {
        out8[a1 ? L.o : dmy] = (uint8_t)e1;
        if (kP1)
            (out8 + 1)[a2 ? L.o : dmy - 1u] = (uint8_t)lut_sym1<kTab>(e1);
        else
            out8[a2 ? L.o + 1 : dmy] = (uint8_t)lut_sym1<kTab>(e1);
    } else {
        if (a1) put8(out8, L.o, e1, L.oend, kStore);
        if (a2) put8(out8, L.o + 1, lut_sym1<kTab>(e1), L.oend, kStore);
    }
    L.o += (uint32_t)a1 + (uint32_t)a2;
    {
        const bool cont = a1 & (a2 | lut_nottwo<kTab>(e1));
        const uint32_t w2 = w << u1;
        const uint32_t rem2 = rem - u1;
        const uint32_t e2 = lut[w2 >> (32 - HPK_LUT_BITS)];
        bool b1, b2;
        const uint32_t u2 = lut12<kTab>(e2, rem2, b1, b2);
        park |= cont & !b1 & (rem2 > (uint32_t)HPK_LUT_BITS);
        b1 &= cont;
        b2 &= cont;
        more2 = b1 & (b2 | lut_nottwo<kTab>(e2));
        if (kStore == kPred) {
            out8[b1 ? L.o : dmy] = (uint8_t)e2;
            if (kP1)
                (out8 + 1)[b2 ? L.o : dmy - 1u] = (uint8_t)lut_sym1<kTab>(e2);
            else
                out8[b2 ? L.o + 1 : dmy] = (uint8_t)lut_sym1<kTab>(e2);
        } else {
            if (b1) put8(out8, L.o, e2, L.oend, kStore);
            if (b2) put8(out8, L.o + 1, lut_sym1<kTab>(e2), L.oend, kStore);
        }
        L.o += (uint32_t)b1 + (uint32_t)b2;
        use += cont ? u2 : 0u;
    }
    const uint32_t xn = L.X + use;
    const bool cross = (xn ^ L.X) > 31u;
    L.d0 = cross ? L.d1 : L.d0;
    L.d1 = cross ? L.d2 : L.d1;
    L.d2 = cross ? d3 : L.d2;
    L.X = xn;
    L.prog = a1 | park;
    if (kMore) L.more = park | more2;
    return park;
}

template <int kStore, bool kMore>
__device__ __forceinline__ void lit12_park(Lit12& L, const uint32_t* __restrict__ win32, const uint16_t* __restrict__ lo,
                                           uint8_t* __restrict__ out8) {
    const uint32_t wp = __builtin_amdgcn_alignbit(L.d0, L.d1, ~L.X);
    uint32_t s, len;
    bool eos;
    lo_decode(wp, lo, s, len, eos);
    const uint32_t r = L.Eb - L.X;
    if (len > r) {
        L.st = HPK_PADDING_TOO_LARGE;
        L.Eb = L.X;
        if (kMore) L.more = false;
    } else if (eos) {
        L.st = HPK_EOS_IN_STRING;
        L.Eb = L.X;
        if (kMore) L.more = false;
    } else {
        put8(out8, L.o, s, L.oend, kStore);
        L.o += 1;
        L.X += len;
        lit12_load(L, win32);
    }
}

template <int kStore, bool kP1 = false,
          int kTab = 2,
          bool kMore = false>
__device__ __forceinline__ void lit12_step(Lit12& L, const uint32_t* __restrict__ win32, const uint32_t* __restrict__ lut,
                                           const uint16_t* __restrict__ lo, uint8_t* __restrict__ out8,
                                           uint32_t dmy = 0) {
    if (lit12_step_main<kStore, kP1, kTab, kMore>(L, win32, lut, out8, dmy)) lit12_park<kStore, kMore>(L, win32, lo, out8);
}

#ifndef HPK_BODY_MIN
#define HPK_BODY_MIN 29
#endif
constexpr uint32_t kBodyMin = HPK_BODY_MIN;

#ifndef HPK_LDS_AS
#define HPK_LDS_AS __attribute__((address_space(3)))
#endif
template <int kStore, int kTab = 2, int kDup = 0>
__device__ __forceinline__ void lit12_body(Lit12& L, const uint32_t* __restrict__ win32, const uint32_t* __restrict__ lut,
                                           const uint16_t* __restrict__ lo, uint8_t* __restrict__ out8, bool& body) {
    const uint32_t d3 = win32[(L.X >> 5) + 2];
    if (kDup == 2) asm volatile("" ::"v"(((const volatile HPK_LDS_AS uint32_t*)win32)[(L.X >> 5) + 2]));
    const uint32_t w = __builtin_amdgcn_alignbit(L.d0, L.d1, ~L.X);
    const uint32_t e1 = lut[w >> (32 - HPK_LUT_BITS)];
    const uint32_t u1 = kTab == 3 ? HPK_L3_HELD(e1) : HPK_L2_HELD(e1);
    const uint32_t e2 = lut[(w << u1) >> (32 - HPK_LUT_BITS)];
    if (kDup == 1) {
        const volatile HPK_LDS_AS uint32_t* vl = (const volatile HPK_LDS_AS uint32_t*)lut;
        asm volatile("" ::"v"(vl[w >> (32 - HPK_LUT_BITS)]));
        asm volatile("" ::"v"(vl[(w << u1) >> (32 - HPK_LUT_BITS)]));
    }
    const uint32_t u2 = kTab == 3 ? HPK_L3_HELD(e2) : HPK_L2_HELD(e2);
    const uint32_t o1 = L.o + (kTab == 3 ? HPK_L3_CODES(e1) : HPK_L2_CODES(e1));
    if (kStore != kNoStore) {
        if (kDup == 3) {
            volatile HPK_LDS_AS uint8_t* v8 = (volatile HPK_LDS_AS uint8_t*)out8;
            v8[L.o] = (uint8_t)e1;
            (v8 + 1)[L.o] = (uint8_t)lut_sym1<kTab>(e1);
            v8[o1] = (uint8_t)e2;
            (v8 + 1)[o1] = (uint8_t)lut_sym1<kTab>(e2);
        }
        out8[L.o] = (uint8_t)e1;
        (out8 + 1)[L.o] = (uint8_t)lut_sym1<kTab>(e1);
        out8[o1] = (uint8_t)e2;
        (out8 + 1)[o1] = (uint8_t)lut_sym1<kTab>(e2);
    }
    L.o = o1 + (kTab == 3 ? HPK_L3_CODES(e2) : HPK_L2_CODES(e2));
    const uint32_t xn = L.X + u1 + u2;
    const bool cross = (xn ^ L.X) > 31u;
    L.d0 = cross ? L.d1 : L.d0;
    L.d1 = cross ? L.d2 : L.d1;
    L.d2 = cross ? d3 : L.d2;
    L.X = xn;
    if (u2 == 0u) {
        const uint32_t wp = __builtin_amdgcn_alignbit(L.d0, L.d1, ~L.X);
        uint32_t sy, len;
        bool eos;
        lo_decode(wp, lo, sy, len, eos);
        const uint32_t r = L.Eb - L.X;
        if (len > r) {
            L.st = HPK_PADDING_TOO_LARGE;
            L.Eb = L.X;
        } else if (eos) {
            L.st = HPK_EOS_IN_STRING;
            L.Eb = L.X;
        } else {
            if (kStore != kNoStore) out8[L.o] = (uint8_t)sy;
            L.o += 1;
            L.X += len;
            lit12_load(L, win32);
        }
    }
    body = L.Eb - L.X >= kBodyMin;
}

struct Tail12 {
    uint32_t n;
    uint32_t used;
    uint32_t o;
    uint32_t rem;
};

__device__ __forceinline__ void tail12_begin(Tail12& T, const Lit12& L) {
    T.rem = L.Eb - L.X;
    T.n = ~__builtin_amdgcn_alignbit(L.d0, L.d1, ~L.X) & ~(0xFFFFFFFFu >> T.rem);
    T.used = 0;
    T.o = L.o;
}

template <int kStore, int kTab>
__device__ __forceinline__ void tail12_look(Tail12& T, const uint32_t* __restrict__ lut, uint8_t* __restrict__ out8,
                                            uint32_t dmy) {
    const uint32_t e = lut[(T.n >> (32 - HPK_LUT_BITS)) ^ (HPK_LUT_SIZE - 1u)];
    const uint32_t held = kTab == 3 ? HPK_L3_HELD(e) : HPK_L2_HELD(e);
    T.used += held;
    const uint32_t codes = T.used <= T.rem ? (kTab == 3 ? HPK_L3_CODES(e) : HPK_L2_CODES(e)) : 0u;
    if (kStore != kNoStore) {
        out8[codes >= 1u ? T.o : dmy] = (uint8_t)e;
        (out8 + 1)[codes >= 2u ? T.o : dmy - 1u] = (uint8_t)lut_sym1<kTab>(e);
    }
    T.o += codes;
    T.n <<= held;
}

__device__ __forceinline__ bool tail12_end(const Tail12& T, Lit12& L) {
    const uint32_t r = T.rem - T.used;
    const bool slow = r > (uint32_t)HPK_LUT_BITS;
    const uint32_t st = r == 0u ? HPK_OK : (r > 7u ? HPK_PADDING_TOO_LARGE : (T.n != 0u ? HPK_INVALID_PADDING : HPK_OK));
    L.X = slow ? L.X : L.X + T.used;
    L.o = slow ? L.o : T.o;
    L.st = slow || L.st != HPK_OK ? L.st : st;
    L.Eb = slow ? L.Eb : L.X;
    return slow;
}

template <int kStore, int kTab>
__device__ __forceinline__ bool lit12_tail(Lit12& L, const uint32_t* __restrict__ lut, uint8_t* __restrict__ out8,
                                           uint32_t dmy) {
    Tail12 T;
    tail12_begin(T, L);
#pragma unroll
    for (int i = 0; i < 4; ++i) tail12_look<kStore, kTab>(T, lut, out8, dmy);
    return tail12_end(T, L);
}

__device__ __forceinline__ uint32_t lit12_status(const Lit12& L) {
    if (L.st != HPK_OK) return L.st;
    return residual_status(L.Eb - L.X, __builtin_amdgcn_alignbit(L.d0, L.d1, ~L.X));
}


struct Lit {
    uint64_t win;
    uint32_t nb;
    uint32_t nxt;
    uint32_t pf;
    uint32_t q;
    uint32_t rem;
    uint32_t cnt;
    uint32_t st;
    uint64_t acc;
    uint32_t accn;
    bool live;
};

struct LdsSwapSrc {
    const uint32_t* p;
    __device__ __forceinline__ uint32_t operator()(uint32_t i) const { return __builtin_bswap32(p[i]); }
};
struct GlobalSrc {
    const uint32_t* p;
    uint32_t last;
    __device__ __forceinline__ uint32_t operator()(uint32_t i) const { return p[min(i, last)]; }
};

template <class Src>
__device__ __forceinline__ void lit_begin(Lit& L, const Src& src, uint32_t sb, uint32_t nbytes) {
    L.rem = nbytes * 8u;
    L.cnt = 0;
    L.st = HPK_OK;
    L.live = nbytes != 0;
    L.acc = 0;
    L.accn = 0;
    const uint32_t q0 = sb >> 2;
    const uint32_t sk = (sb & 3u) * 8u;
    const uint32_t d0 = src(q0);
    L.nxt = src(q0 + 1);
    L.pf = src(q0 + 2);
    L.q = q0 + 2;
    L.win = ((uint64_t)__builtin_bswap32(d0) << 32) << sk;
    L.nb = 32u - sk;
}

template <class Src>
__device__ __forceinline__ void lit_refill(Lit& L, const Src& src) {
    const bool need = L.nb <= 32u;
    const uint64_t add = (uint64_t)__builtin_bswap32(L.nxt) << ((32u - L.nb) & 63u);
    L.win |= need ? add : 0ull;
    L.nb += need ? 32u : 0u;
    L.nxt = need ? L.pf : L.nxt;
    L.q += need ? 1u : 0u;
    L.pf = src(L.q);
}

template <class Src, class Dst>
__device__ __forceinline__ void lit_bytes_to(Lit& L, const Src& src, const uint16_t* lo, Dst dst, uint32_t ocap,
                                             uint32_t sb, uint32_t nbytes) {
    lit_begin(L, src, sb, nbytes);
    while (L.live) {
        lit_refill(L, src);
        uint32_t sym, len;
        bool eos;
        lo_decode((uint32_t)(L.win >> 32), lo, sym, len, eos);
        if (len > L.rem) break;
        if (eos) {
            L.st = HPK_EOS_IN_STRING;
            break;
        }
        if (L.cnt >= ocap) {
            L.st = HPK_OUTPUT_OVERFLOW;
            break;
        }
        dst(L.cnt, (uint8_t)sym);
        L.cnt += 1;
        L.win <<= len;
        L.nb -= len;
        L.rem -= len;
        L.live = L.rem != 0u;
    }
}

__device__ __forceinline__ uint32_t lit_status(const Lit& L) {
    uint32_t st = L.st;
    if (st == HPK_OK && L.rem > 0) {
        if (L.rem > 7) {
            st = HPK_PADDING_TOO_LARGE;
        } else {
            const uint32_t w = (uint32_t)(L.win >> 32) | (0xFFFFFFFFu >> L.rem);
            if (w != 0xFFFFFFFFu) st = HPK_INVALID_PADDING;
        }
    }
    return st;
}

}
```

loona_amd/csrc/hpk_wave.h:

```cpp
#pragma once
#include <type_traits>

#include "hpk_decode_kernel.h"
#include "hpk_huge.h"
#include "hpk_long.h"

#ifndef HPK_BODY_UNROLL
#define HPK_BODY_UNROLL 4
#endif
#ifndef HPK_LUT3
#define HPK_LUT3 1
#endif
#ifndef HPK_CW_LANE_DIAG
#define HPK_CW_LANE_DIAG 0
#endif
#ifndef HPK_NT_STORE
#define HPK_NT_STORE 1
#endif
#ifndef HPK_NT_LOAD
#define HPK_NT_LOAD 1
#endif
#ifndef HPK_TAIL_MASKED
#define HPK_TAIL_MASKED 1
#endif
#ifndef HPK_WIN_CUT
#define HPK_WIN_CUT 1
#endif

namespace hpkdec {

typedef uint32_t v4u32 __attribute__((ext_vector_type(4)));
__device__ __forceinline__ void st16(uint4* p, const uint4 v) {
    if (HPK_NT_STORE) {
        const v4u32 x = {v.x, v.y, v.z, v.w};
        __builtin_nontemporal_store(x, reinterpret_cast<v4u32*>(p));
    } else {
        *p = v;
    }
}
__device__ __forceinline__ uint4 ld16(const uint4* p) {
    if (HPK_NT_LOAD) {
        const v4u32 x = __builtin_nontemporal_load(reinterpret_cast<const v4u32*>(p));
        return make_uint4(x.x, x.y, x.z, x.w);
    }
    return *p;
}

template <int kWinB, int kImgB>
struct GeoW {
    static constexpr int kWaves = 16, kBlock = kWaves * 64;
    static constexpr int kWaveBytes = kWinB + kImgB;
    static constexpr int kLutOff = kTabBytes;
    static constexpr int kWaveOff = kTabBytes + (int)HPK_LUT_SIZE * 4;
    static constexpr int kCtrOff = kWaveOff + kWaves * kWaveBytes;
    static constexpr int kLdsBytes = kCtrOff + 64 + (int)kHugeMax * 4;
    static constexpr int kImg = kImgB - 256;
    static constexpr int kWinRounds = (kWinB / 16 + 63) / 64;
    static constexpr int kFlushRounds = (kImg / 16 + 1 + 63) / 64;
    static_assert(kLdsBytes <= 163840, "LDS budget (160 KiB per CU on gfx950)");
    static_assert(kWinB % 16 == 0 && kImgB % 16 == 0 && kWinB < 65536 && kImgB < 131072, "entry packing");
    static_assert(kWaves * kWaveBytes >= huge_lds_bytes<kBlock>(), "huge-phase LDS");
};

__device__ __forceinline__ uint32_t wave_incl_scan(uint32_t x, uint32_t lane) {
    x += (uint32_t)__builtin_amdgcn_update_dpp(0, (int)x, 0x111, 0xF, 0xF, false);
    x += (uint32_t)__builtin_amdgcn_update_dpp(0, (int)x, 0x112, 0xF, 0xF, false);
    x += (uint32_t)__builtin_amdgcn_update_dpp(0, (int)x, 0x114, 0xF, 0xF, false);
    x += (uint32_t)__builtin_amdgcn_update_dpp(0, (int)x, 0x118, 0xF, 0xF, false);
    const uint32_t r0 = (uint32_t)__builtin_amdgcn_readlane((int)x, 15);
    const uint32_t r1 = (uint32_t)__builtin_amdgcn_readlane((int)x, 31);
    const uint32_t r2 = (uint32_t)__builtin_amdgcn_readlane((int)x, 47);
    return x + (lane >= 16u ? r0 : 0u) + (lane >= 32u ? r1 : 0u) + (lane >= 48u ? r2 : 0u);
}

template <int kMode, int kWinB, int kImgB, uint32_t kChunk, int kGuided, int kRank, bool kCompact = false>
__global__ __launch_bounds__(1024) void hpk_decode_wave(DecodeArgs a) {
    using G = GeoW<kWinB, kImgB>;
    constexpr int kStore = kMode == 2 ? kNoStore : kPred;
    constexpr uint32_t kStamps = 13;
    __shared__ uint32_t s_dg[kMode == 3 ? G::kWaves * kStamps : 1];
    uint32_t tq = kMode == 3 ? (uint32_t)__builtin_amdgcn_s_memtime() : 0u;
    const uint32_t t_start = tq;
    auto dg_add = [&](int i, uint32_t v) {
        if (kMode == 3 && (threadIdx.x & 63u) == 0u) atomicAdd(&s_dg[(threadIdx.x >> 6) * kStamps + i], v);
    };
    auto stamp = [&](int i) {
        if (kMode == 3) {
            const uint32_t t = (uint32_t)__builtin_amdgcn_s_memtime();
            dg_add(i, t - tq);
            tq = t;
        }
    };
    constexpr int R = G::kWinRounds, F = G::kFlushRounds;
    __shared__ __attribute__((aligned(16))) uint8_t smem[G::kLdsBytes];
    uint16_t* s_lo = reinterpret_cast<uint16_t*>(smem + kT8Bytes);
    uint32_t* s_lut = reinterpret_cast<uint32_t*>(smem + G::kLutOff);
    uint32_t* s_ctr = reinterpret_cast<uint32_t*>(smem + G::kCtrOff);
    uint32_t* s_huge = s_ctr + 16;
    const uint32_t tid = threadIdx.x, lane = tid & 63u, wv = tid >> 6;
    constexpr int kTab = HPK_LUT3 ? 3 : 2;
    const uint32_t BA = (uint32_t)((uint64_t)a.n * blockIdx.x / gridDim.x);
    const uint32_t BB = (uint32_t)((uint64_t)a.n * (blockIdx.x + 1) / gridDim.x);
    static_assert(G::kBlock == 1024, "the dense check's two offsets rounds");
    const uint32_t c0 = kGuided == 2 ? kChunk : max(kChunk, (BB - BA) / 32u);
    const uint32_t cur0 = kGuided == 0 ? BA + (uint32_t)((uint64_t)(BB - BA) * wv / G::kWaves) : min(BA + wv * c0, BB);
    const uint32_t ce0 =
        kGuided == 0 ? BA + (uint32_t)((uint64_t)(BB - BA) * (wv + 1) / G::kWaves) : min(cur0 + c0, BB);
    const uint32_t gin0 = a.in_off[cur0];
    const uint32_t gend0 = HPK_WIN_CUT ? a.in_off[ce0] : 0u;
    const uint32_t gout0 = kCompact ? 0u : a.out_off[cur0];
    const uint32_t kd = min(BB - BA, 2048u);
    uint32_t dv0[2], dv1[2];
#pragma unroll
    for (int r = 0; r < 2; ++r) {
        const uint32_t tt = BA + min(tid + (uint32_t)G::kBlock * r, kd ? kd - 1u : 0u);
        dv0[r] = a.in_off[tt];
        dv1[r] = a.in_off[tt + 1u];
    }
    for (uint32_t t = tid; t < kLoBytes / 16; t += G::kBlock)
        reinterpret_cast<uint4*>(s_lo)[t] = reinterpret_cast<const uint4*>(a.lo)[t];
    for (uint32_t t = tid; t < HPK_LUT_SIZE * 4 / 16; t += G::kBlock)
        reinterpret_cast<uint4*>(s_lut)[t] = reinterpret_cast<const uint4*>(kTab == 3 ? a.lut3 : a.lut2)[t];
    if (tid < 16) s_ctr[tid] = tid == 7 && kGuided ? min(G::kWaves * c0, BB - BA) : 0u;
    if (kMode == 3)
        for (uint32_t t = tid; t < (uint32_t)G::kWaves * kStamps; t += G::kBlock) s_dg[t] = 0;
    const uint32_t in_end = min(a.in_off[a.n], a.in_cap) + a.in_mis;
    const uint32_t last16 = in_end ? (in_end - 1) >> 4 : 0;
    const uint32_t in0 = kCompact ? a.in_off[0] : 0u;
    auto ulay = [&](uint32_t i, uint32_t io) -> uint32_t {
        const uint32_t d = io - in0, q = __umulhi(d, 0xCCCCCCCDu) >> 2;
        return d + 3u * q + (((d - 5u * q) * 39u) >> 6) + 4u * i;
    };
    auto oof = [&](uint32_t i) -> uint32_t { return kCompact ? ulay(i, a.in_off[i]) : a.out_off[i]; };
    if (kCompact && blockIdx.x == 0 && tid == 0) a.co_off[a.n] = ulay(a.n, a.in_off[a.n]);
    const uint32_t wg0 = kCompact && BA < BB ? oof(BA) : 0u;
    auto leave = [&](uint32_t i, uint32_t nb) {
        if (kCompact) a.co_off[i] = wg0 + atomicAdd(&s_ctr[9], ((nb * 8u) / 5u + 3u) & ~3u);
        if (nb >= HPK_HUGE_MIN && nb < kHugeLimit) {
            const uint32_t h = atomicAdd(&s_ctr[8], 1u);
            if (h < kHugeMax) {
                s_huge[h] = i;
                return;
            }
        }
        if (nb >= a.long_big)
            a.long_list[BA + atomicAdd(&s_ctr[1], 1u)] = i;
        else
            a.long_list[BB - 1u - atomicAdd(&s_ctr[2], 1u)] = i;
    };
    __syncthreads();
    bool dense = false;
    {
        uint32_t dlb = 0, dtb = 0;
#pragma unroll
        for (int r = 0; r < 2; ++r) {
            if (tid + (uint32_t)G::kBlock * r < kd) {
                const uint32_t nb = min(dv1[r] - dv0[r], 1u << 20);
                dtb += nb;
                dlb += nb >= a.long_min ? nb : 0u;
            }
        }
#pragma unroll
        for (int d = 32; d >= 1; d >>= 1) {
            dlb += __shfl_xor(dlb, d);
            dtb += __shfl_xor(dtb, d);
        }
        if (lane == 0 && dtb) {
            atomicAdd(&s_ctr[4], dlb);
            atomicAdd(&s_ctr[5], dtb);
        }
        __syncthreads();
        if (s_ctr[4] > s_ctr[5] / 2u) {
            uint32_t* const s_cls = reinterpret_cast<uint32_t*>(smem + G::kWaveOff);
            if (tid < 64) s_cls[tid] = 0;
            __syncthreads();
            bool no = false;
            for (uint32_t i = BA + tid; i < BB; i += G::kBlock) {
                const uint32_t p0 = a.in_off[i], p1 = a.in_off[i + 1];
                const uint32_t q0 = kCompact ? ulay(i, p0) : a.out_off[i], q1 = kCompact ? ulay(i + 1u, p1) : a.out_off[i + 1];
                const bool ok = p0 <= p1 && p1 <= a.in_cap && q0 <= q1 && q1 <= a.out_cap &&
                                (uint64_t)(q1 - q0) >= (uint64_t)(p1 - p0) * 8u / 5u;
                if (!ok) {
                    no = true;
                    continue;
                }
                const uint32_t nb = p1 - p0;
                if (!(nb >= HPK_HUGE_MIN && nb < kHugeLimit)) atomicAdd(&s_cls[lpt_class_of(nb)], 1u);
            }
            if (__any(no) && lane == 0) s_ctr[6] = 1u;
            __syncthreads();
            dense = s_ctr[6] == 0u;
            if (dense) {
                if (tid < 64) {
                    const uint32_t v = tid < 32 ? s_cls[tid] : 0u;
                    uint32_t x = v;
#pragma unroll
                    for (int d = 1; d < 64; d <<= 1) {
                        const uint32_t y = __shfl_up(x, d);
                        if (lane >= (uint32_t)d) x += y;
                    }
                    if (tid < 32) s_cls[32 + tid] = x - v;
                    if (tid == 31) s_ctr[1] = x;
                }
                __syncthreads();
                for (uint32_t i = BA + tid; i < BB; i += G::kBlock) {
                    const uint32_t nb = a.in_off[i + 1] - a.in_off[i];
                    if (kCompact) a.co_off[i] = wg0 + atomicAdd(&s_ctr[9], ((nb * 8u) / 5u + 3u) & ~3u);
                    bool huge = false;
                    if (nb >= HPK_HUGE_MIN && nb < kHugeLimit) {
                        const uint32_t hh = atomicAdd(&s_ctr[8], 1u);
                        if (hh < kHugeMax) {
                            s_huge[hh] = i;
                            huge = true;
                        }
                    }
                    if (!huge)
                        a.long_list[nb >= HPK_HUGE_MIN && nb < kHugeLimit ? BB - 1u - atomicAdd(&s_ctr[2], 1u)
                                                                          : BA + atomicAdd(&s_cls[32 + lpt_class_of(nb)], 1u)] = i;
                }
                __syncthreads();
            }
            if (!dense) {
                __syncthreads();
                if (tid == 0) {
                    s_ctr[1] = 0;
                    s_ctr[2] = 0;
                    s_ctr[8] = 0;
                    s_ctr[9] = 0;
                }
                __syncthreads();
            }
        }
    }
    if (!dense) {
        uint8_t* const s_win = smem + G::kWaveOff + wv * G::kWaveBytes;
        uint8_t* const s_img = s_win + kWinB;
        const uint32_t* const win32 = reinterpret_cast<const uint32_t*>(s_win);
        const uint32_t wbits = (uint32_t)(G::kWaveOff + wv * G::kWaveBytes) * 8u;
        const uint32_t obase = (uint32_t)(G::kWaveOff + wv * G::kWaveBytes + kWinB);
        const uint32_t* const wl32 = reinterpret_cast<const uint32_t*>(smem);
        uint8_t* const ol8 = smem;
        const uint32_t dmy = obase + (uint32_t)G::kImg + lane * 4u;
        bool given = false;
        auto claim = [&](uint32_t& ca, uint32_t& ce) {
            if (!kGuided) {
                ca = given ? BB : BA + (uint32_t)((uint64_t)(BB - BA) * wv / G::kWaves);
                ce = given ? BB : BA + (uint32_t)((uint64_t)(BB - BA) * (wv + 1) / G::kWaves);
                given = true;
                return;
            }
            uint32_t c = 0;
            if (lane == 0) {
                const uint32_t seen = *(volatile HPK_LDS_AS uint32_t*)(&s_ctr[7]);
                const uint32_t left = BB - BA > seen ? BB - BA - seen : 0u;
                const uint32_t want = kGuided == 2 ? kChunk : max(kChunk, left / 32u);
                c = atomicAdd(&s_ctr[7], want);
                c = c < BB - BA ? c : BB - BA;
                ce = BA + min(c + want, BB - BA);
            }
            ca = BA + (uint32_t)__builtin_amdgcn_readfirstlane((int)c);
            ce = (uint32_t)__builtin_amdgcn_readfirstlane((int)ce);
        };
        uint32_t io0[2], oo0[2], ie = 0, oe = 0, pcnt = 1, pc = 0;
        uint4 ch[R];
        constexpr bool kCut = HPK_WIN_CUT != 0;
        constexpr uint32_t kWinC = (uint32_t)kWinB / 16u;
        auto chunk_lim = [&](uint32_t x) {
            x = min(x, a.in_cap) + a.in_mis;
            return min(last16, x ? (x - 1u) >> 4 : 0u);
        };
        uint32_t clim = kCut ? chunk_lim(gend0) : last16;
        auto prefetch = [&](uint32_t c, uint32_t e, uint32_t base16) {
            const uint32_t cnt = min(128u, e - c);
#pragma unroll
            for (int r = 0; r < 2; ++r) {
                const uint32_t t = c + min(lane + 64u * r, cnt - 1u);
                io0[r] = a.in_off[t];
                if (!kCompact) oo0[r] = a.out_off[t];
            }
            ie = a.in_off[c + cnt];
            if (!kCompact) oe = a.out_off[c + cnt];
            pcnt = cnt;
            pc = c;
            const uint4* g16 = reinterpret_cast<const uint4*>(a.in_base);
#pragma unroll
            for (int r = 0; r < R; ++r) ch[r] = ld16(g16 + min((base16 >> 4) + lane + 64u * r, clim));
        };
        uint32_t io1[2], oo1[2];
        auto ends = [&]() {
            if (kCompact) {
#pragma unroll
                for (int r = 0; r < 2; ++r) oo0[r] = ulay(pc + min(lane + 64u * r, pcnt - 1u), io0[r]);
                oe = ulay(pc + pcnt, ie);
            }
            const uint32_t i1 = (uint32_t)__builtin_amdgcn_readfirstlane((int)io0[1]);
            const uint32_t o1 = (uint32_t)__builtin_amdgcn_readfirstlane((int)oo0[1]);
#pragma unroll
            for (int r = 0; r < 2; ++r) {
                const uint32_t ni = (uint32_t)__builtin_amdgcn_update_dpp((int)(r ? ie : i1), (int)io0[r], 0x130, 0xF, 0xF, false);
                const uint32_t no = (uint32_t)__builtin_amdgcn_update_dpp((int)(r ? oe : o1), (int)oo0[r], 0x130, 0xF, 0xF, false);
                const bool last = lane + 64u * r + 1u >= pcnt;
                io1[r] = last ? ie : ni;
                oo1[r] = last ? oe : no;
            }
        };
        uint32_t cur = cur0, ce = ce0;
        given = true;
        uint32_t gin = 0, gout = 0;
        uint32_t sens[4] = {0u, 1u, 2u, 3u};
        if (cur < ce) {
            gin = gin0 + a.in_mis;
            gout = (kCompact ? ulay(cur, gin0) : gout0) + a.out_mis;
            prefetch(cur, ce, gin & ~15u);
        }
        uint32_t pk = 0, pcur = 0, pG0 = 0, pG1 = 0;
        uint32_t rv0 = 0, rv1 = 0, ri0 = 0xFFFFFFFFu, ri1 = 0xFFFFFFFFu;
        uint32_t stop = 0;
        stamp(11);
        auto opaque = [](uint32_t x) {
            asm volatile("" : "+v"(x));
            return x;
        };
        auto flush = [&]() {
            const uint32_t ob = pG0 & ~15u;
            const uint32_t c0 = ob >> 4, c1 = (pG1 + 15u) >> 4;
            uint4* l16 = reinterpret_cast<uint4*>(s_img) + (opaque(lane) - lane);
            uint4* g16 = reinterpret_cast<uint4*>(a.out_base);
            if (kMode != 2) {
                if (lane < 32) {
                    const uint32_t g = lane < 16 ? c0 << 4 : (c1 - 1u) << 4;
                    const bool partial = !(g >= pG0 && g + 16u <= pG1) && (lane < 16 || c1 - 1u != c0);
                    const uint32_t x = g + (lane & 15u);
                    if (partial && x >= pG0 && x < pG1) a.out_base[x] = s_img[x - ob];
                }
#pragma unroll
                for (int r = 0; r < F; ++r) {
                    const uint32_t ci = c0 + lane + 64u * r;
                    if (ci < c1) {
                        if ((ci << 4) >= pG0 && (ci << 4) + 16u <= pG1) st16(g16 + ci, l16[ci - c0]);
                    }
                }
            }
            if (ri0 != 0xFFFFFFFFu) {
                a.out_len[pcur + ri0] = rv0 & 0xFFFFFFu;
                a.status[pcur + ri0] = (uint8_t)(rv0 >> 24);
            }
            if (ri1 != 0xFFFFFFFFu) {
                a.out_len[pcur + ri1] = rv1 & 0xFFFFFFu;
                a.status[pcur + ri1] = (uint8_t)(rv1 >> 24);
            }
            ri0 = ri1 = 0xFFFFFFFFu;
        };
        auto compact_fill = [&](uint32_t fcur, uint32_t fk, const uint2 q1, const uint2 q2) {
            uint32_t* const s_len = reinterpret_cast<uint32_t*>(s_win);
            uint32_t* const s_ex = s_len + 128;
            static_assert(256 * 4 <= kWinB, "compact tables in the window");
            s_len[lane] = kListed;
            s_len[lane + 64u] = kListed;
            if (ri0 != 0xFFFFFFFFu) s_len[ri0] = rv0;
            if (ri1 != 0xFFFFFFFFu) s_len[ri1] = rv1;
            const uint32_t l0 = s_len[lane], l1 = s_len[lane + 64u];
            const uint32_t x0 = l0 == kListed ? 0u : l0 & 0xFFFFFFu, x1 = l1 == kListed ? 0u : l1 & 0xFFFFFFu;
            const uint32_t i0 = wave_incl_scan(x0, lane), i1 = wave_incl_scan(x1, lane);
            const uint32_t t0 = (uint32_t)__builtin_amdgcn_readlane((int)i0, 63);
            const uint32_t ex0 = i0 - x0, ex1 = t0 + i1 - x1;
            const uint32_t tot = t0 + (uint32_t)__builtin_amdgcn_readlane((int)i1, 63);
            uint32_t u = 0;
            if (lane == 0) u = atomicAdd(&s_ctr[9], tot);
            const uint32_t base = wg0 + (uint32_t)__builtin_amdgcn_readfirstlane((int)u);
            if (tot != 0u) {
                const uint32_t D0 = a.out_mis + base;
                s_ex[lane] = ex0;
                s_ex[lane + 64u] = ex1;
                __builtin_amdgcn_wave_barrier();
                const uint32_t* const img32 = reinterpret_cast<const uint32_t*>(s_img);
                uint32_t js[2], jd[2], jn[2];
#pragma unroll
                for (int r = 0; r < 2; ++r) {
                    const uint32_t ri = r ? ri1 : ri0, rv = r ? rv1 : rv0;
                    const bool on = ri != 0xFFFFFFFFu && rv != kListed;
                    js[r] = ((r ? q2.y : q1.y) >> 12) & 0x1FFFFu;
                    jd[r] = D0 + s_ex[on ? ri : 0u];
                    jn[r] = on ? rv & 0xFFFFFFu : 0u;
                }
                auto dw_at = [&](uint32_t u) {
                    return __builtin_amdgcn_alignbyte(img32[(u >> 2) + 1u], img32[u >> 2], u & 3u);
                };
                uint32_t sp = js[0], dp = jd[0], np = jn[0], tp = 0;
                bool second = true;
                if (np == 0u) {
                    sp = js[1];
                    dp = jd[1];
                    np = jn[1];
                    second = false;
                }
                while (HPK_CW_LANE_DIAG != 2 && __any(tp < np)) {
                    if (tp < np) {
                        if (np >= 16u) {
                            const uint32_t t = min(tp, np - 16u), u = sp + t;
                            const uint32_t sw = u >> 2, s3 = u & 3u;
                            uint32_t A[5];
#pragma unroll
                            for (int j = 0; j < 5; ++j) A[j] = img32[sw + (uint32_t)j];
                            u32x4u v;
                            v.x = __builtin_amdgcn_alignbyte(A[1], A[0], s3);
                            v.y = __builtin_amdgcn_alignbyte(A[2], A[1], s3);
                            v.z = __builtin_amdgcn_alignbyte(A[3], A[2], s3);
                            v.w = __builtin_amdgcn_alignbyte(A[4], A[3], s3);
                            if (HPK_CW_LANE_DIAG == 3)
                                *reinterpret_cast<u32x4u*>(a.out_base + ((dp + t) & ~15u)) = v;
                            else if (HPK_CW_LANE_DIAG == 4)
                                asm volatile("" ::"v"(v.x), "v"(v.y), "v"(v.z), "v"(v.w));
                            else
                                *reinterpret_cast<u32x4u*>(a.out_base + dp + t) = v;
                            tp += 16u;
                        } else if (np >= 4u) {
                            u32u* const g = reinterpret_cast<u32u*>(a.out_base + dp);
                            g[0] = dw_at(sp);
                            if (np >= 8u) g[1] = dw_at(sp + 4u);
                            if (np >= 12u) g[2] = dw_at(sp + 8u);
                            *reinterpret_cast<u32u*>(a.out_base + dp + np - 4u) = dw_at(sp + np - 4u);
                            tp = np;
                        } else {
                            for (uint32_t b = 0; b < np; ++b) a.out_base[dp + b] = s_img[sp + b];
                            tp = np;
                        }
                        if (tp >= np && second) {
                            sp = js[1];
                            dp = jd[1];
                            np = jn[1];
                            tp = 0;
                            second = false;
                        }
                    }
                }
            }
            if (lane < fk && l0 != kListed) {
                a.co_off[fcur + lane] = base + ex0;
                a.out_len[fcur + lane] = x0;
                a.status[fcur + lane] = (uint8_t)(l0 >> 24);
            }
            if (lane + 64u < fk && l1 != kListed) {
                a.co_off[fcur + lane + 64u] = base + ex1;
                a.out_len[fcur + lane + 64u] = x1;
                a.status[fcur + lane + 64u] = (uint8_t)(l1 >> 24);
            }
        };
        while (cur < ce) {
            const uint32_t cntl = min(128u, ce - cur);
            const uint32_t base16 = gin & ~15u, ob16 = gout & ~15u;
            bool bad = false;
            uint32_t ex[2], ey[2];
            bool fits[2];
            ends();
#pragma unroll
            for (int r = 0; r < 2; ++r) {
                const uint32_t t = lane + 64u * r;
                bad |= t < cntl && !(io0[r] <= io1[r] && io1[r] <= a.in_cap && oo0[r] <= oo1[r] && oo1[r] <= a.out_cap);
                const uint32_t p0 = io0[r] + a.in_mis, p1 = io1[r] + a.in_mis;
                const uint32_t o0 = oo0[r] + a.out_mis, o1 = oo1[r] + a.out_mis;
                fits[r] = t < cntl && p1 - base16 <= (uint32_t)kWinB && o1 - ob16 <= (uint32_t)G::kImg;
                const uint32_t nbytes = p1 - p0, ocap = o1 - o0;
                const bool fast = ocap >= (nbytes * 8u) / 5u;
                ex[r] = (p0 - base16) | (nbytes << 16);
                ey[r] = t | ((o0 - ob16) << 12) | (fast ? 0u : kQ7Byte);
            }
            const bool wbad = __any(bad) || stop != 0u;
            stamp(1);
            dg_add(8, 1u);
            if (wbad) {
                if (pk) flush();
                pk = 0;
                if (lane == 0) {
                    *a.err = 1u;
                    s_ctr[0] = 1u;
                }
                for (;;) {
                    for (uint32_t i = cur + lane; i < ce; i += 64u) {
                        a.out_len[i] = 0;
                        a.status[i] = (uint8_t)HPK_BAD_OFFSETS;
                    }
                    claim(cur, ce);
                    if (cur >= ce) break;
                }
                break;
            }
            const uint64_t f0 = __ballot(fits[0]), f1 = __ballot(fits[1]);
            const uint32_t k = (uint32_t)__popcll(f0) + (uint32_t)__popcll(f1);
            if (k == 0) {
                if (pk) flush();
                pk = 0;
                const uint32_t nb = a.in_off[cur + 1] - a.in_off[cur];
                const bool left = nb >= a.long_min && oof(cur + 1) - oof(cur) >= (nb * 8u) / 5u;
                if (lane == 0) {
                    if (left) {
                        leave(cur, nb);
                    } else {
                        const GlobalSrc g{reinterpret_cast<const uint32_t*>(a.in_base), last16 * 4 + 3};
                        uint8_t* dst = a.out_base + gout;
                        if (kCompact) {
                            const uint32_t o = wg0 + atomicAdd(&s_ctr[9], ((nb * 8u) / 5u + 3u) & ~3u);
                            a.co_off[cur] = o;
                            dst = a.out_base + a.out_mis + o;
                        }
                        Lit L = {};
                        lit_bytes_to(L, g, s_lo, [&](uint32_t j, uint8_t v) { dst[j] = v; },
                                     oof(cur + 1) - oof(cur), gin, a.in_off[cur + 1] + a.in_mis - gin);
                        a.out_len[cur] = L.cnt;
                        a.status[cur] = (uint8_t)lit_status(L);
                    }
                }
                cur += 1;
                if (cur == ce) {
                    claim(cur, ce);
                    if (kCut && cur < ce) clim = chunk_lim(a.in_off[ce]);
                }
                if (cur < ce) {
                    gin = a.in_off[cur] + a.in_mis;
                    gout = oof(cur) + a.out_mis;
                    prefetch(cur, ce, gin & ~15u);
                }
                continue;
            }
            const uint64_t fl = f1 ? f1 : f0;
            const int hl = 63 - __builtin_clzll(fl);
            const uint32_t gin_end = (uint32_t)__builtin_amdgcn_readlane((int)((f1 ? io1[1] : io1[0]) + a.in_mis), hl);
            const uint32_t gout_end =
                (uint32_t)__builtin_amdgcn_readlane((int)((f1 ? oo1[1] : oo1[0]) + a.out_mis), hl);
            uint32_t cur_n = cur + k, ce_n = ce, gin_n = gin_end, gout_n = gout_end;
            if (cur_n == ce) {
                claim(cur_n, ce_n);
                if (cur_n < ce_n) {
                    gin_n = a.in_off[cur_n] + a.in_mis;
                    gout_n = oof(cur_n) + a.out_mis;
                    if (kCut) clim = chunk_lim(a.in_off[ce_n]);
                }
            }
            {
                uint4* l16 = reinterpret_cast<uint4*>(s_win) + (opaque(lane) - lane);
#pragma unroll
                for (int r = 0; r < R; ++r) {
                    const uint4 c = ch[r];
                    const uint32_t j = lane + 64u * r;
                    if (j < kWinC)
                        l16[j] = make_uint4(__builtin_bswap32(c.x), __builtin_bswap32(c.y), __builtin_bswap32(c.z),
                                            __builtin_bswap32(c.w));
                }
            }
            stamp(4);
            if (pk) flush();
            stamp(2);
            bool qd[2];
            uint32_t key[2];
#pragma unroll
            for (int r = 0; r < 2; ++r) {
                const uint32_t nbytes = ex[r] >> 16;
                const bool lng = nbytes >= a.long_min && !(ey[r] & kQ7Byte);
                if (fits[r] && lng) leave(cur + lane + 64u * r, nbytes);
                qd[r] = fits[r] && !lng;
                key[r] = kRank == 1 ? min(nbytes >> 2, 15u) : min(nbytes >> 1, 31u);
            }
            uint32_t rank0 = 0, rank1 = 0, kq = 0;
            uint2* const q = reinterpret_cast<uint2*>(s_img + 256);
            if (kRank == 0) {
                uint32_t* const hist = reinterpret_cast<uint32_t*>(s_img);
                if (lane < 32) hist[lane] = 0;
                const uint32_t pa = qd[0] ? atomicAdd(&hist[31u - key[0]], 1u) : 0u;
                const uint32_t pb = qd[1] ? atomicAdd(&hist[31u - key[1]], 1u) : 0u;
                const uint32_t v = lane < 32 ? hist[lane] : 0u;
                uint32_t x = v;
                x += (uint32_t)__builtin_amdgcn_update_dpp(0, (int)x, 0x111, 0xF, 0xF, false);
                x += (uint32_t)__builtin_amdgcn_update_dpp(0, (int)x, 0x112, 0xF, 0xF, false);
                x += (uint32_t)__builtin_amdgcn_update_dpp(0, (int)x, 0x114, 0xF, 0xF, false);
                x += (uint32_t)__builtin_amdgcn_update_dpp(0, (int)x, 0x118, 0xF, 0xF, false);
                const uint32_t row0 = (uint32_t)__builtin_amdgcn_readlane((int)x, 15);
                x += lane >= 16u ? row0 : 0u;
                if (lane < 32) hist[32 + lane] = x - v;
                kq = (uint32_t)__builtin_amdgcn_readlane((int)x, 31);
                rank0 = qd[0] ? hist[32 + 31 - key[0]] + pa : 0u;
                rank1 = qd[1] ? hist[32 + 31 - key[1]] + pb : 0u;
            }
#pragma unroll
            for (int c = (kRank == 1 ? 15 : 31); kRank != 0 && c >= 0; --c) {
                const bool h0 = qd[0] && key[0] == (uint32_t)c, h1 = qd[1] && key[1] == (uint32_t)c;
                const uint64_t m0 = __ballot(h0), m1 = __ballot(h1);
                const uint32_t p0 = (uint32_t)__popcll(m0);
                const uint32_t b0 = __builtin_amdgcn_mbcnt_hi((uint32_t)(m0 >> 32), __builtin_amdgcn_mbcnt_lo((uint32_t)m0, 0u));
                const uint32_t b1 = __builtin_amdgcn_mbcnt_hi((uint32_t)(m1 >> 32), __builtin_amdgcn_mbcnt_lo((uint32_t)m1, 0u));
                rank0 = h0 ? kq + b0 : rank0;
                rank1 = h1 ? kq + p0 + b1 : rank1;
                kq += p0 + (uint32_t)__popcll(m1);
            }
            if (qd[0]) q[rank0] = make_uint2(ex[0], ey[0]);
            if (qd[1]) q[rank1] = make_uint2(ex[1], ey[1]);
            stamp(3);
            const uint32_t t1 = lane, t2 = 127u - lane;
            const uint2 e1 = kq ? q[min(t1, kq - 1u)] : make_uint2(0u, 0u);
            const uint2 e2 = kq ? q[min(t2, kq - 1u)] : make_uint2(0u, 0u);
            stop = *(volatile HPK_LDS_AS uint32_t*)(&s_ctr[0]);
            {
                const bool more = cur_n < ce_n;
                prefetch(more ? cur_n : cur, more ? ce_n : cur + k, (more ? gin_n : gin) & ~15u);
            }
            Lit12 L, N;
            auto load = [&](Lit12& T, const uint2 e, uint32_t tt) {
                T.act = tt < kq && !(e.y & kQ7Byte);
                T.idx = e.y & 0xFFFu;
                const uint32_t nb = e.x >> 16;
                const uint32_t o = (e.y >> 12) & 0x1FFFFu;
                T.X = wbits + (e.x & 0xFFFFu) * 8u + 31u;
                T.Eb = T.X + (T.act ? nb * 8u : 0u);
                T.o = obase + o;
                T.o0 = obase + o;
                T.st = HPK_OK;
                T.prog = false;
                lit12_load(T, wl32);
            };
            load(L, e1, t1);
            uint32_t sX = 0, sO = 0, sSt = 0;
            bool s1 = false;
            stamp(5);
            uint32_t Lend = 0;
            if (kMode != 1) {
                bool body = L.Eb - L.X >= kBodyMin;
                uint32_t aX = L.X, aO = L.o, aSt = L.st;
                bool aAct = L.act, onA = true;
                for (;;) {
                    dg_add(9, 1u);
#pragma unroll
                    for (int s = 0; s < HPK_BODY_UNROLL; ++s) {
                        if (body)
                            lit12_body<kStore, kTab, (kMode >= 8 && kMode <= 10) ? kMode - 7 : 0>(L, wl32, s_lut, s_lo, ol8,
                                                                                                   body);
                        if (kMode == 6) {
#pragma unroll
                            for (int q = 0; q < 4; ++q) {
                                asm volatile("v_xor_b32 %0, %0, %1" : "+v"(sens[0]) : "v"(L.X));
                                asm volatile("v_xor_b32 %0, %0, %1" : "+v"(sens[1]) : "v"(L.o));
                                asm volatile("v_xor_b32 %0, %0, %1" : "+v"(sens[2]) : "v"(L.Eb));
                                asm volatile("v_xor_b32 %0, %0, %1" : "+v"(sens[3]) : "v"(L.d1));
                            }
                        }
                    }
                    if (__any(!body)) {
                        const bool sw = !body & onA;
                        if (sw) {
                            aX = L.X;
                            aO = L.o;
                            aSt = L.st;
                            aAct = L.act;
                            load(L, e2, t2);
                            onA = false;
                            body = L.Eb - L.X >= kBodyMin;
                        }
                        if (!__any(body)) break;
                    }
                }
                N = L;
                L.X = aX;
                L.o = aO;
                L.st = aSt;
                L.act = aAct;
                L.Eb = wbits + (e1.x & 0xFFFFu) * 8u + 31u + (aAct ? (e1.x >> 16) * 8u : 0u);
                L.o0 = obase + ((e1.y >> 12) & 0x1FFFFu);
                L.idx = e1.y & 0xFFFu;
                if (aSt != HPK_OK) L.Eb = L.X;
                lit12_load(L, wl32);
                L.more = L.Eb - L.X >= 5u;
                N.more = N.Eb - N.X >= 5u;
                stamp(12);
                if (HPK_TAIL_MASKED) {
                    Tail12 TL, TN;
                    tail12_begin(TL, L);
                    tail12_begin(TN, N);
#pragma unroll
                    for (int s = 0; s < 4; ++s) {
                        tail12_look<kStore, kTab>(TL, s_lut, ol8, dmy);
                        tail12_look<kStore, kTab>(TN, s_lut, ol8, dmy);
                    }
                    L.more &= tail12_end(TL, L);
                    N.more &= tail12_end(TN, N);
                }
                while (__any(L.more | N.more)) {
                    if (L.more) lit12_step<kStore, true, kTab, true>(L, wl32, s_lut, s_lo, ol8, dmy);
                    if (N.more) lit12_step<kStore, true, kTab, true>(N, wl32, s_lut, s_lo, ol8, dmy);
                }
                sX = L.X;
                sO = L.o;
                sSt = L.st;
                s1 = L.act;
                L = N;
                Lend = L.o;
            }
            stamp(6);
            if (kMode == 6 && (sens[0] ^ sens[1] ^ sens[2] ^ sens[3]) == 0x5EB51u)
                a.status[0] = 9u;
            {
                const uint32_t Eb = wbits + (e1.x & 0xFFFFu) * 8u + 31u + (e1.x >> 16) * 8u;
                const uint32_t st = sSt != HPK_OK ? sSt : residual_status(Eb - sX, win_at(wl32, sX - 31u));
                rv0 = (sO - obase - ((e1.y >> 12) & 0x1FFFFu)) | (st << 24);
                ri0 = s1 ? e1.y & 0xFFFu : 0xFFFFFFFFu;
                rv1 = (Lend - L.o0) | (lit12_status(L) << 24);
                ri1 = L.act ? L.idx : 0xFFFFFFFFu;
            }
            if (kMode == 1) {
                rv0 = 0;
                ri0 = t1 < kq ? e1.y & 0xFFFu : 0xFFFFFFFFu;
            }
#pragma unroll
            for (int r = 0; r < 2; ++r) {
                const uint2 e = r == 0 ? e1 : e2;
                const uint32_t tt = r == 0 ? t1 : t2;
                if (tt < kq && (e.y & kQ7Byte)) {
                    const uint32_t i = e.y & 0xFFFu;
                    const uint32_t o = (e.y >> 12) & 0x1FFFFu;
                    Lit B = {};
                    lit_bytes_to(B, LdsSwapSrc{win32}, s_lo, [&](uint32_t j, uint8_t v) { s_img[o + j] = v; },
                                 oof(cur + i + 1) - oof(cur + i), e.x & 0xFFFFu, e.x >> 16);
                    if (r == 0) {
                        rv0 = B.cnt | (lit_status(B) << 24);
                        ri0 = i;
                    } else {
                        rv1 = B.cnt | (lit_status(B) << 24);
                        ri1 = i;
                    }
                }
            }
            stamp(7);
            if (kCompact) {
#pragma unroll
                for (int r = 0; r < 2; ++r) asm volatile("" ::"v"(io0[r]), "s"(ie));
#pragma unroll
                for (int r = 0; r < R; ++r) asm volatile("" ::"v"(ch[r].x), "v"(ch[r].y), "v"(ch[r].z), "v"(ch[r].w));
                compact_fill(cur, k, e1, e2);
            } else {
                pk = k;
                pcur = cur;
                pG0 = gout;
                pG1 = gout_end;
            }
            cur = cur_n;
            ce = ce_n;
            gin = gin_n;
            gout = gout_n;
        }
        if (pk) flush();
        stamp(2);
    }
    __syncthreads();
    const uint32_t c1 = s_ctr[1], c2 = s_ctr[2], nh = min(s_ctr[8], kHugeMax);
    huge_phase<G::kBlock, kTab>(a, s_huge, nh, reinterpret_cast<uint32_t*>(smem + G::kWaveOff), s_lut, s_lo);
    if (c1 + c2) {
        static_assert(G::kWaveOff % 16 == 0, "long-phase rings");
        uint8_t* const area = smem + G::kWaveOff;
        constexpr int kLB = HPK_LONG_WAVES * 64;
        constexpr int kLQ = kLB * (HPK_LONG_RING * 4 + HPK_LONG_OS);
        static_assert(kLQ + HPK_LONG_WAVES * HPK_LONG_CLAIM * 16 <= G::kWaves * G::kWaveBytes, "long-phase LDS");
        long_phase<kLB, HPK_LONG_U, HPK_LONG_RING, kMode == 5 ? 1 : 0, G::kBlock, HPK_LONG_OS, HPK_LONG_CLAIM, kTab>(
            a, BA, BB, c1, c2, &s_ctr[3], reinterpret_cast<uint32_t*>(area), area + kLB * HPK_LONG_RING * 4,
            reinterpret_cast<uint4*>(area + kLQ), s_lut, s_lo);
    }
    stamp(10);
    if (kMode == 3) {
        __syncthreads();
        if (lane < kStamps) {
            const uint32_t v = lane == 0 ? (uint32_t)__builtin_amdgcn_s_memtime() - t_start : s_dg[wv * kStamps + lane];
            a.dbg[((uint64_t)blockIdx.x * G::kWaves + wv) * 16u + lane] = v;
        }
    }
}

}
```

Before: 1141.

## Decode wave fills with a 13-bit two-symbol LDS lookup table

Adds a 13-bit two-symbol lookup table, built and validated against the 12-bit table on the host, and makes it the default for the wave-fill kernel. More codes and symbol pairs now resolve in one LDS lookup, so fewer steps fall back to the slow path. In exchange the table doubles to 32 KiB of LDS, so the per-wave window and image sizes are retuned, the dummy store slot moves to a shared carve-out, and the unused t8 and 12-bit lut device tables are dropped. The body threshold rises to 31 bits, which leaves more bits to the checked tail steps.

```diff
diff --git a/loona_amd/csrc/hpk_code.h b/loona_amd/csrc/hpk_code.h
--- a/loona_amd/csrc/hpk_code.h
+++ b/loona_amd/csrc/hpk_code.h
@@ -5,6 +5,8 @@
 #define HPK_EOS 256
 #define HPK_LUT_BITS 12
 #define HPK_LUT_SIZE (1u << HPK_LUT_BITS)
+#define HPK_LUT13_BITS 13
+#define HPK_LUT13_SIZE (1u << HPK_LUT13_BITS)
 #define HPK_LO_RUNS 30
 #define HPK_LO_SIZE (HPK_LO_RUNS * 32)
 
@@ -54,6 +56,7 @@
     uint32_t lut[HPK_LUT_SIZE];
     uint32_t lut2[HPK_LUT_SIZE];
     uint32_t lut3[HPK_LUT_SIZE];
+    uint32_t lut13[HPK_LUT13_SIZE];
     uint16_t lo[HPK_LO_SIZE];
     uint8_t t8[256];
 };
@@ -135,5 +138,30 @@
         t->lut3[v] = (e2 & 0xFFu) | (HPK_L2_HELD(e2) << 8) | (e2 & 0x00FF0000u) | (codes << 24) |
                      ((codes ? HPK_L2_LEN0(e2) : 15u) << 26) | (codes < 2 ? HPK_L3_NOTTWO : 0u);
     }
+    for (uint32_t v = 0; v < HPK_LUT13_SIZE; ++v) {
+        const uint32_t w = v << (32 - HPK_LUT13_BITS);
+        int s0 = -1, l0 = 0, s1 = -1, l1 = 0;
+        for (int s = 0; s < 256; ++s) {
+            int L = t->len[s];
+            if (L <= HPK_LUT13_BITS && (w >> (32 - L)) == t->code[s]) { s0 = s; l0 = L; break; }
+        }
+        if (s0 < 0) {
+            t->lut13[v] = (15u << 26) | HPK_L3_NOTTWO;
+        } else {
+            const uint32_t w1 = w << l0;
+            const int rem = HPK_LUT13_BITS - l0;
+            for (int s = 0; s < 256 && rem >= 5; ++s) {
+                int L = t->len[s];
+                if (L <= rem && (w1 >> (32 - L)) == t->code[s]) { s1 = s; l1 = L; break; }
+            }
+            t->lut13[v] = (uint32_t)s0 | ((uint32_t)(l0 + l1) << 8) | ((uint32_t)(s1 < 0 ? 0 : s1) << 16) |
+                          ((s1 < 0 ? 1u : 2u) << 24) | ((uint32_t)l0 << 26) | (s1 < 0 ? HPK_L3_NOTTWO : 0u);
+        }
+        const uint32_t e = t->lut13[v], e3 = t->lut3[v >> 1];
+        if (HPK_L3_HELD(e) > HPK_LUT13_BITS) return -1;
+        if (HPK_L3_CODES(e3) == 2u && e != e3) return -1;
+        if (HPK_L3_CODES(e3) == 1u && ((e & 0xFFu) != (e3 & 0xFFu) || HPK_L3_LEN0(e) != HPK_L3_LEN0(e3))) return -1;
+        if (HPK_L3_CODES(e3) == 0u && HPK_L3_CODES(e) != 0u && HPK_L3_LEN0(e) != HPK_LUT13_BITS) return -1;
+    }
     return 0;
 }
diff --git a/loona_amd/csrc/hpk_ctx.hip b/loona_amd/csrc/hpk_ctx.hip
--- a/loona_amd/csrc/hpk_ctx.hip
+++ b/loona_amd/csrc/hpk_ctx.hip
@@ -6,7 +6,7 @@
 
 #include "hpk_device.h"
 
-#define HPK_VERSION "hpk 0.38 gfx950 decode v38 (every batch: wave fills, each wave with its own LDS window and image, longest-first queue, slot end offsets by DPP, nontemporal window loads stopping at the chunk's last byte, nontemporal write-back; chunks by guided self-scheduling from 4M literals, fixed 96-literal chunks below; fills and long-literal phase: body steps with no fit tests while >= 29 bits are left, then the wave fills' tails as four masked lookups with no fit test per code (checked steps only for a 13..28-bit code or a cut code in the tail) and the other kernels' checked tails (the long phase's at its refill points); long literals one lane each streaming from HBM after the fills, dense ranges listed longest-first; literals of >= 8 KiB by a whole workgroup in speculative pieces; compacted-output form: wave fills packed per workgroup from an LDS cursor into a bound layout made from the input offsets, each lane storing its two literals in unaligned 16-byte pieces; small-call mode: a persistent kernel behind a host-mapped doorbell); encode v5 (byte-balanced workgroup ranges, start map and DPP segmented scan, run accumulator, LDS image, live chunks only)"
+#define HPK_VERSION "hpk 0.39 gfx950 decode v39 (every batch: wave fills, each wave with its own LDS window and image, lookups in a 13-bit two-symbol table, longest-first queue, slot end offsets by DPP, nontemporal window loads stopping at the chunk's last byte, nontemporal write-back; chunks by guided self-scheduling from 4M literals, fixed 96-literal chunks below; fills and long-literal phase: body steps with no fit tests while >= 31 bits are left (29 with the 12-bit table), then the wave fills' tails as four masked lookups with no fit test per code (checked steps only for a 14..30-bit code or a cut code in the tail) and the other kernels' checked tails (the long phase's at its refill points); long literals one lane each streaming from HBM after the fills, dense ranges listed longest-first; literals of >= 8 KiB by a whole workgroup in speculative pieces; compacted-output form: wave fills packed per workgroup from an LDS cursor into a bound layout made from the input offsets, each lane storing its two literals in unaligned 16-byte pieces; small-call mode: a persistent kernel behind a host-mapped doorbell); encode v5 (byte-balanced workgroup ranges, start map and DPP segmented scan, run accumulator, LDS image, live chunks only)"
 
 static thread_local std::string t_last_error;
 
@@ -52,17 +52,16 @@
     c->num_cu = prop.multiProcessorCount;
     if ((e = hipStreamCreateWithFlags(&c->own, hipStreamNonBlocking)) != hipSuccess) return fail("hipStreamCreate", e);
     c->stream = c->own;
-    if ((e = hipMalloc(&c->d_lut, sizeof(t->lut))) != hipSuccess) return fail("hipMalloc lut", e);
-    if ((e = hipMemcpy(c->d_lut, t->lut, sizeof(t->lut), hipMemcpyHostToDevice)) != hipSuccess) return fail("upload lut", e);
     if ((e = hipMalloc(&c->d_lut2, sizeof(t->lut2))) != hipSuccess) return fail("hipMalloc lut2", e);
     if ((e = hipMemcpy(c->d_lut2, t->lut2, sizeof(t->lut2), hipMemcpyHostToDevice)) != hipSuccess)
         return fail("upload lut2", e);
     if ((e = hipMalloc(&c->d_lut3, sizeof(t->lut3))) != hipSuccess) return fail("hipMalloc lut3", e);
     if ((e = hipMemcpy(c->d_lut3, t->lut3, sizeof(t->lut3), hipMemcpyHostToDevice)) != hipSuccess)
         return fail("upload lut3", e);
+    if ((e = hipMalloc(&c->d_lut13, sizeof(t->lut13))) != hipSuccess) return fail("hipMalloc lut13", e);
+    if ((e = hipMemcpy(c->d_lut13, t->lut13, sizeof(t->lut13), hipMemcpyHostToDevice)) != hipSuccess)
+        return fail("upload lut13", e);
     if ((e = hipMalloc(&c->d_lo, sizeof(t->lo))) != hipSuccess) return fail("hipMalloc lo", e);
-    if ((e = hipMalloc(&c->d_t8, sizeof(t->t8))) != hipSuccess) return fail("hipMalloc t8", e);
-    if ((e = hipMemcpy(c->d_t8, t->t8, sizeof(t->t8), hipMemcpyHostToDevice)) != hipSuccess) return fail("upload t8", e);
     if ((e = hipMalloc(&c->d_codes, 2 * 257 * sizeof(uint32_t))) != hipSuccess) return fail("hipMalloc codes", e);
     uint32_t packed[2 * 257];
     for (int s = 0; s < 257; ++s) {
@@ -153,11 +152,10 @@
     if (c->h_sm) (void)hipHostFree(c->h_sm);
     (void)hipFree(c->d_sm_dev);
     (void)hipStreamSynchronize(c->stream);
-    (void)hipFree(c->d_lut);
     (void)hipFree(c->d_lut2);
     (void)hipFree(c->d_lut3);
+    (void)hipFree(c->d_lut13);
     (void)hipFree(c->d_lo);
-    (void)hipFree(c->d_t8);
     (void)hipFree(c->d_codes);
     (void)hipFree(c->d_in);
     (void)hipFree(c->d_out);
diff --git a/loona_amd/csrc/hpk_decode.hip b/loona_amd/csrc/hpk_decode.hip
--- a/loona_amd/csrc/hpk_decode.hip
+++ b/loona_amd/csrc/hpk_decode.hip
@@ -16,7 +16,13 @@
 #define HPK_LONG_BIG 1024
 #endif
 using Geo = Geo12<kWaves, kW, kO, kQ>;
-constexpr int kWaveWin = 3072, kWaveImg = 5888;
+#ifndef HPK_WAVE_WIN
+#define HPK_WAVE_WIN 3008
+#endif
+#ifndef HPK_WAVE_IMG
+#define HPK_WAVE_IMG (8048 - HPK_WAVE_WIN)
+#endif
+constexpr int kWaveWin = HPK_WAVE_WIN, kWaveImg = HPK_WAVE_IMG;
 #ifndef HPK_WAVE_MIN
 #define HPK_WAVE_MIN 0u
 #endif
@@ -79,11 +85,10 @@
     a.out_off = b.out_off;
     a.out_len = b.out_len;
     a.status = b.status;
-    a.t8 = c->d_t8;
     a.lo = c->d_lo;
-    a.lut = c->d_lut;
     a.lut2 = c->d_lut2;
     a.lut3 = c->d_lut3;
+    a.lut13 = c->d_lut13;
     a.dbg = nullptr;
     a.in_cap = b.in_cap;
     a.out_cap = b.out_cap;
diff --git a/loona_amd/csrc/hpk_decode_kernel.h b/loona_amd/csrc/hpk_decode_kernel.h
--- a/loona_amd/csrc/hpk_decode_kernel.h
+++ b/loona_amd/csrc/hpk_decode_kernel.h
@@ -20,11 +20,10 @@
     const uint32_t* out_off;
     uint32_t* out_len;
     uint8_t* status;
-    const uint8_t* t8;
     const uint16_t* lo;
-    const uint32_t* lut;
     const uint32_t* lut2;
     const uint32_t* lut3;
+    const uint32_t* lut13;
     unsigned long long* dbg;
     uint32_t in_cap, out_cap;
     uint32_t* err;
diff --git a/loona_amd/csrc/hpk_device.h b/loona_amd/csrc/hpk_device.h
--- a/loona_amd/csrc/hpk_device.h
+++ b/loona_amd/csrc/hpk_device.h
@@ -42,11 +42,10 @@
     int decode_kernel = HPK_DECODE_AUTO;
     hipStream_t own = nullptr;
     hipStream_t stream = nullptr;
-    uint32_t* d_lut = nullptr;
     uint32_t* d_lut2 = nullptr;
     uint32_t* d_lut3 = nullptr;
+    uint32_t* d_lut13 = nullptr;
     uint16_t* d_lo = nullptr;
-    uint8_t* d_t8 = nullptr;
     uint32_t* d_codes = nullptr;
     uint8_t* d_in = nullptr;
     size_t d_in_cap = 0;
diff --git a/loona_amd/csrc/hpk_huge_piece.h b/loona_amd/csrc/hpk_huge_piece.h
--- a/loona_amd/csrc/hpk_huge_piece.h
+++ b/loona_amd/csrc/hpk_huge_piece.h
@@ -57,14 +57,14 @@
         }
     }
     const uint32_t w = (uint32_t)(W.win >> 32);
-    const uint32_t e = lut[w >> (32 - HPK_LUT_BITS)];
-    const uint32_t l0 = kTab == 3 ? HPK_L3_LEN0(e) : HPK_L2_LEN0(e);
-    if (l0 <= (uint32_t)HPK_LUT_BITS) {
+    const uint32_t e = lut[w >> (32 - lut_bits<kTab>())];
+    const uint32_t l0 = lut_l3<kTab>() ? HPK_L3_LEN0(e) : HPK_L2_LEN0(e);
+    if (l0 <= lut_bits<kTab>()) {
         sym = e & 0xFFu;
         len = l0;
         eos = false;
-        const uint32_t codes = kTab == 3 ? HPK_L3_CODES(e) : HPK_L2_CODES(e);
-        held = codes == 2u ? (kTab == 3 ? HPK_L3_HELD(e) : HPK_L2_HELD(e)) : 0u;
+        const uint32_t codes = lut_l3<kTab>() ? HPK_L3_CODES(e) : HPK_L2_CODES(e);
+        held = codes == 2u ? (lut_l3<kTab>() ? HPK_L3_HELD(e) : HPK_L2_HELD(e)) : 0u;
         sym1 = (e >> 16) & 0xFFu;
     } else {
         lo_decode(w, lo, sym, len, eos);
diff --git a/loona_amd/csrc/hpk_long.h b/loona_amd/csrc/hpk_long.h
--- a/loona_amd/csrc/hpk_long.h
+++ b/loona_amd/csrc/hpk_long.h
@@ -70,6 +70,7 @@
     constexpr uint32_t kQ = kChunk;
     static_assert(kClaim == 32 || kClaim == 64, "claim size");
     constexpr uint32_t kOS = kOSz;
+    static_assert(body_min<kTab>() <= 35u, "a tail's bytes");
     static_assert(15 + 5 * kU + 3 + (HPK_LONG_TAILPT ? 6 : 0) < (int)kOS, "output buffer");
     static_assert((kRing & (kRing - 1)) == 0 && kRing >= 16 && 4 * kCh + 8 <= kRing, "input ring: a power of two >= 16 dwords");
     static_assert(kBlock % 64 == 0 && kBlock <= kBlockAll, "decoding waves");
@@ -122,23 +123,23 @@
         }
         if (HPK_LONG_TAILPT) {
             for (;;) {
-                const bool tl = act && live && !done && Eb - X < kBodyMin && h * 4u >= span;
+                const bool tl = act && live && !done && Eb - X < body_min<kTab>() && h * 4u >= span;
                 if (!__any(tl)) break;
                 if (tl) {
                     const uint32_t j0 = X >> 5;
                     const uint32_t d3 = ring[((j0 + 2u) & (kRing - 1u)) * kBlock];
                     const uint32_t w = __builtin_amdgcn_alignbit(d0, d1, ~X);
                     const uint32_t rem = Eb - X;
-                    const uint32_t e1 = s_lut[w >> (32 - HPK_LUT_BITS)];
+                    const uint32_t e1 = s_lut[w >> (32 - lut_bits<kTab>())];
                     bool a1, a2;
                     const uint32_t u1 = lut12<kTab>(e1, rem, a1, a2);
-                    bool park = !a1 & (rem > (uint32_t)HPK_LUT_BITS);
+                    bool park = !a1 & (rem > lut_bits<kTab>());
                     const bool cont = a1 & (a2 | lut_nottwo<kTab>(e1));
                     const uint32_t rem2 = rem - u1;
-                    const uint32_t e2 = s_lut[(w << u1) >> (32 - HPK_LUT_BITS)];
+                    const uint32_t e2 = s_lut[(w << u1) >> (32 - lut_bits<kTab>())];
                     bool b1, b2;
                     const uint32_t v2 = lut12<kTab>(e2, rem2, b1, b2);
-                    park |= cont & !b1 & (rem2 > (uint32_t)HPK_LUT_BITS);
+                    park |= cont & !b1 & (rem2 > lut_bits<kTab>());
                     b1 &= cont;
                     b2 &= cont;
                     const uint32_t g1 = (uint32_t)a1 + (uint32_t)a2, g2 = (uint32_t)b1 + (uint32_t)b2;
@@ -325,7 +326,7 @@
                                 : h * 4u >= span ? (uint32_t)kU
                                 : x5 + 4u <= h ? min((uint32_t)kU, ((h - x5 - 4u) >> 1) + 1u) : 0u;
         for (int s = 0; s < kU; ++s) {
-            const bool go = (uint32_t)s < budget && !done && (!HPK_LONG_TAILPT || Eb - X >= kBodyMin);
+            const bool go = (uint32_t)s < budget && !done && (!HPK_LONG_TAILPT || Eb - X >= body_min<kTab>());
             if (kDiag) {
                 dg[2] += (unsigned long long)__popcll(__ballot(go));
                 dg[3] += (unsigned long long)__popcll(__ballot(act && live && !done && !go));
@@ -340,27 +341,27 @@
             const uint32_t rem = Eb - X;
             uint32_t e1, e2, u1, u2, g1, g2;
             bool park, prog;
-            if (HPK_LONG_TAILPT || (HPK_LONG_BODY && rem >= kBodyMin)) {
-                e1 = s_lut[w >> (32 - HPK_LUT_BITS)];
-                u1 = kTab == 3 ? HPK_L3_HELD(e1) : HPK_L2_HELD(e1);
-                e2 = s_lut[(w << u1) >> (32 - HPK_LUT_BITS)];
-                u2 = kTab == 3 ? HPK_L3_HELD(e2) : HPK_L2_HELD(e2);
-                g1 = kTab == 3 ? HPK_L3_CODES(e1) : HPK_L2_CODES(e1);
-                g2 = kTab == 3 ? HPK_L3_CODES(e2) : HPK_L2_CODES(e2);
+            if (HPK_LONG_TAILPT || (HPK_LONG_BODY && rem >= body_min<kTab>())) {
+                e1 = s_lut[w >> (32 - lut_bits<kTab>())];
+                u1 = lut_l3<kTab>() ? HPK_L3_HELD(e1) : HPK_L2_HELD(e1);
+                e2 = s_lut[(w << u1) >> (32 - lut_bits<kTab>())];
+                u2 = lut_l3<kTab>() ? HPK_L3_HELD(e2) : HPK_L2_HELD(e2);
+                g1 = lut_l3<kTab>() ? HPK_L3_CODES(e1) : HPK_L2_CODES(e1);
+                g2 = lut_l3<kTab>() ? HPK_L3_CODES(e2) : HPK_L2_CODES(e2);
                 park = u2 == 0u;
                 prog = true;
             } else {
-                e1 = s_lut[w >> (32 - HPK_LUT_BITS)];
+                e1 = s_lut[w >> (32 - lut_bits<kTab>())];
                 bool a1, a2;
                 u1 = lut12<kTab>(e1, rem, a1, a2);
-                park = !a1 & (rem > (uint32_t)HPK_LUT_BITS);
+                park = !a1 & (rem > lut_bits<kTab>());
                 const bool cont = a1 & (a2 | lut_nottwo<kTab>(e1));
                 const uint32_t w2 = w << u1;
                 const uint32_t rem2 = rem - u1;
-                e2 = s_lut[w2 >> (32 - HPK_LUT_BITS)];
+                e2 = s_lut[w2 >> (32 - lut_bits<kTab>())];
                 bool b1, b2;
                 const uint32_t v2 = lut12<kTab>(e2, rem2, b1, b2);
-                park |= cont & !b1 & (rem2 > (uint32_t)HPK_LUT_BITS);
+                park |= cont & !b1 & (rem2 > lut_bits<kTab>());
                 b1 &= cont;
                 b2 &= cont;
                 g1 = (uint32_t)a1 + (uint32_t)a2;
diff --git a/loona_amd/csrc/hpk_walk.h b/loona_amd/csrc/hpk_walk.h
--- a/loona_amd/csrc/hpk_walk.h
+++ b/loona_amd/csrc/hpk_walk.h
@@ -42,10 +42,21 @@
     return __builtin_amdgcn_alignbit(q[-1], q[0], ~x);
 }
 
+template <int kTab>
+constexpr uint32_t lut_bits() {
+    static_assert(kTab >= 2 && kTab <= 4, "table kind");
+    return kTab == 4 ? (uint32_t)HPK_LUT13_BITS : (uint32_t)HPK_LUT_BITS;
+}
+template <int kTab>
+constexpr bool lut_l3() {
+    return kTab >= 3;
+}
+
 template <int kTab = 2>
 __device__ __forceinline__ uint32_t lut12(uint32_t e, uint32_t rem, bool& ok1, bool& ok2) {
+    static_assert(lut_bits<kTab>() < HPK_LUT2_CLAMP, "a held length is below the clamp");
     const uint32_t rc = min(rem, HPK_LUT2_CLAMP);
-    if (kTab == 3) {
+    if (lut_l3<kTab>()) {
         const uint32_t l1 = HPK_L3_LEN0(e), t1 = HPK_L3_HELD(e);
         ok1 = l1 <= rc;
         ok2 = (t1 <= rc) & (e < HPK_L3_NOTTWO);
@@ -58,7 +69,7 @@
 }
 template <int kTab>
 __device__ __forceinline__ bool lut_nottwo(uint32_t e) {
-    return kTab == 3 ? e >= HPK_L3_NOTTWO : e >= HPK_LUT2_NOTTWO;
+    return lut_l3<kTab>() ? e >= HPK_L3_NOTTWO : e >= HPK_LUT2_NOTTWO;
 }
 template <int kTab>
 __device__ __forceinline__ uint32_t lut_sym1(uint32_t e) {
@@ -109,11 +120,11 @@
     const uint32_t d3 = win32[(L.X >> 5) + 2];
     const uint32_t w = __builtin_amdgcn_alignbit(L.d0, L.d1, ~L.X);
     const uint32_t rem = L.Eb - L.X;
-    const uint32_t e1 = lut[w >> (32 - HPK_LUT_BITS)];
+    const uint32_t e1 = lut[w >> (32 - lut_bits<kTab>())];
     bool a1, a2;
     const uint32_t u1 = lut12<kTab>(e1, rem, a1, a2);
     uint32_t use = u1;
-    bool park = !a1 & (rem > (uint32_t)HPK_LUT_BITS);
+    bool park = !a1 & (rem > lut_bits<kTab>());
     bool more2 = false;
     if (kStore == kPred) {
         out8[a1 ? L.o : dmy] = (uint8_t)e1;
@@ -130,10 +141,10 @@
         const bool cont = a1 & (a2 | lut_nottwo<kTab>(e1));
         const uint32_t w2 = w << u1;
         const uint32_t rem2 = rem - u1;
-        const uint32_t e2 = lut[w2 >> (32 - HPK_LUT_BITS)];
+        const uint32_t e2 = lut[w2 >> (32 - lut_bits<kTab>())];
         bool b1, b2;
         const uint32_t u2 = lut12<kTab>(e2, rem2, b1, b2);
-        park |= cont & !b1 & (rem2 > (uint32_t)HPK_LUT_BITS);
+        park |= cont & !b1 & (rem2 > lut_bits<kTab>());
         b1 &= cont;
         b2 &= cont;
         more2 = b1 & (b2 | lut_nottwo<kTab>(e2));
@@ -198,6 +209,10 @@
 #define HPK_BODY_MIN 29
 #endif
 constexpr uint32_t kBodyMin = HPK_BODY_MIN;
+template <int kTab>
+constexpr uint32_t body_min() {
+    return lut_bits<kTab>() == (uint32_t)HPK_LUT_BITS ? kBodyMin : 2u * lut_bits<kTab>() + 5u;
+}
 
 #ifndef HPK_LDS_AS
 #define HPK_LDS_AS __attribute__((address_space(3)))
@@ -208,16 +223,16 @@
     const uint32_t d3 = win32[(L.X >> 5) + 2];
     if (kDup == 2) asm volatile("" ::"v"(((const volatile HPK_LDS_AS uint32_t*)win32)[(L.X >> 5) + 2]));
     const uint32_t w = __builtin_amdgcn_alignbit(L.d0, L.d1, ~L.X);
-    const uint32_t e1 = lut[w >> (32 - HPK_LUT_BITS)];
-    const uint32_t u1 = kTab == 3 ? HPK_L3_HELD(e1) : HPK_L2_HELD(e1);
-    const uint32_t e2 = lut[(w << u1) >> (32 - HPK_LUT_BITS)];
+    const uint32_t e1 = lut[w >> (32 - lut_bits<kTab>())];
+    const uint32_t u1 = lut_l3<kTab>() ? HPK_L3_HELD(e1) : HPK_L2_HELD(e1);
+    const uint32_t e2 = lut[(w << u1) >> (32 - lut_bits<kTab>())];
     if (kDup == 1) {
         const volatile HPK_LDS_AS uint32_t* vl = (const volatile HPK_LDS_AS uint32_t*)lut;
-        asm volatile("" ::"v"(vl[w >> (32 - HPK_LUT_BITS)]));
-        asm volatile("" ::"v"(vl[(w << u1) >> (32 - HPK_LUT_BITS)]));
-    }
-    const uint32_t u2 = kTab == 3 ? HPK_L3_HELD(e2) : HPK_L2_HELD(e2);
-    const uint32_t o1 = L.o + (kTab == 3 ? HPK_L3_CODES(e1) : HPK_L2_CODES(e1));
+        asm volatile("" ::"v"(vl[w >> (32 - lut_bits<kTab>())]));
+        asm volatile("" ::"v"(vl[(w << u1) >> (32 - lut_bits<kTab>())]));
+    }
+    const uint32_t u2 = lut_l3<kTab>() ? HPK_L3_HELD(e2) : HPK_L2_HELD(e2);
+    const uint32_t o1 = L.o + (lut_l3<kTab>() ? HPK_L3_CODES(e1) : HPK_L2_CODES(e1));
     if (kStore != kNoStore) {
         if (kDup == 3) {
             volatile HPK_LDS_AS uint8_t* v8 = (volatile HPK_LDS_AS uint8_t*)out8;
@@ -231,7 +246,7 @@
         out8[o1] = (uint8_t)e2;
         (out8 + 1)[o1] = (uint8_t)lut_sym1<kTab>(e2);
     }
-    L.o = o1 + (kTab == 3 ? HPK_L3_CODES(e2) : HPK_L2_CODES(e2));
+    L.o = o1 + (lut_l3<kTab>() ? HPK_L3_CODES(e2) : HPK_L2_CODES(e2));
     const uint32_t xn = L.X + u1 + u2;
     const bool cross = (xn ^ L.X) > 31u;
     L.d0 = cross ? L.d1 : L.d0;
@@ -257,7 +272,7 @@
             lit12_load(L, win32);
         }
     }
-    body = L.Eb - L.X >= kBodyMin;
+    body = L.Eb - L.X >= body_min<kTab>();
 }
 
 struct Tail12 {
@@ -277,10 +292,10 @@
 template <int kStore, int kTab>
 __device__ __forceinline__ void tail12_look(Tail12& T, const uint32_t* __restrict__ lut, uint8_t* __restrict__ out8,
                                             uint32_t dmy) {
-    const uint32_t e = lut[(T.n >> (32 - HPK_LUT_BITS)) ^ (HPK_LUT_SIZE - 1u)];
-    const uint32_t held = kTab == 3 ? HPK_L3_HELD(e) : HPK_L2_HELD(e);
+    const uint32_t e = lut[(T.n >> (32 - lut_bits<kTab>())) ^ ((1u << lut_bits<kTab>()) - 1u)];
+    const uint32_t held = lut_l3<kTab>() ? HPK_L3_HELD(e) : HPK_L2_HELD(e);
     T.used += held;
-    const uint32_t codes = T.used <= T.rem ? (kTab == 3 ? HPK_L3_CODES(e) : HPK_L2_CODES(e)) : 0u;
+    const uint32_t codes = T.used <= T.rem ? (lut_l3<kTab>() ? HPK_L3_CODES(e) : HPK_L2_CODES(e)) : 0u;
     if (kStore != kNoStore) {
         out8[codes >= 1u ? T.o : dmy] = (uint8_t)e;
         (out8 + 1)[codes >= 2u ? T.o : dmy - 1u] = (uint8_t)lut_sym1<kTab>(e);
@@ -289,9 +304,10 @@
     T.n <<= held;
 }
 
+template <int kTab = 2>
 __device__ __forceinline__ bool tail12_end(const Tail12& T, Lit12& L) {
     const uint32_t r = T.rem - T.used;
-    const bool slow = r > (uint32_t)HPK_LUT_BITS;
+    const bool slow = r > lut_bits<kTab>();
     const uint32_t st = r == 0u ? HPK_OK : (r > 7u ? HPK_PADDING_TOO_LARGE : (T.n != 0u ? HPK_INVALID_PADDING : HPK_OK));
     L.X = slow ? L.X : L.X + T.used;
     L.o = slow ? L.o : T.o;
@@ -307,7 +323,7 @@
     tail12_begin(T, L);
 #pragma unroll
     for (int i = 0; i < 4; ++i) tail12_look<kStore, kTab>(T, lut, out8, dmy);
-    return tail12_end(T, L);
+    return tail12_end<kTab>(T, L);
 }
 
 __device__ __forceinline__ uint32_t lit12_status(const Lit12& L) {
diff --git a/loona_amd/csrc/hpk_wave.h b/loona_amd/csrc/hpk_wave.h
--- a/loona_amd/csrc/hpk_wave.h
+++ b/loona_amd/csrc/hpk_wave.h
@@ -8,8 +8,8 @@
 #ifndef HPK_BODY_UNROLL
 #define HPK_BODY_UNROLL 4
 #endif
-#ifndef HPK_LUT3
-#define HPK_LUT3 1
+#ifndef HPK_WAVE_TAB
+#define HPK_WAVE_TAB 4
 #endif
 #ifndef HPK_CW_LANE_DIAG
 #define HPK_CW_LANE_DIAG 0
@@ -46,15 +46,18 @@
     return *p;
 }
 
-template <int kWinB, int kImgB>
+template <int kWinB, int kImgB, int kTab>
 struct GeoW {
     static constexpr int kWaves = 16, kBlock = kWaves * 64;
     static constexpr int kWaveBytes = kWinB + kImgB;
-    static constexpr int kLutOff = kTabBytes;
-    static constexpr int kWaveOff = kTabBytes + (int)HPK_LUT_SIZE * 4;
+    static constexpr int kLutBytes = 4 << lut_bits<kTab>();
+    static constexpr int kLutOff = kLoBytes;
+    static constexpr int kDummyOff = kLutOff + kLutBytes;
+    static constexpr int kWaveOff = kDummyOff + 256;
     static constexpr int kCtrOff = kWaveOff + kWaves * kWaveBytes;
     static constexpr int kLdsBytes = kCtrOff + 64 + (int)kHugeMax * 4;
-    static constexpr int kImg = kImgB - 256;
+    static constexpr int kImg = kImgB;
+    static_assert(kLoBytes % 16 == 0, "16-byte aligned carve-outs");
     static constexpr int kWinRounds = (kWinB / 16 + 63) / 64;
     static constexpr int kFlushRounds = (kImg / 16 + 1 + 63) / 64;
     static_assert(kLdsBytes <= 163840, "LDS budget (160 KiB per CU on gfx950)");
@@ -75,7 +78,8 @@
 
 template <int kMode, int kWinB, int kImgB, uint32_t kChunk, int kGuided, int kRank, bool kCompact = false>
 __global__ __launch_bounds__(1024) void hpk_decode_wave(DecodeArgs a) {
-    using G = GeoW<kWinB, kImgB>;
+    constexpr int kTab = HPK_WAVE_TAB;
+    using G = GeoW<kWinB, kMode == 3 ? kImgB - 64 : kImgB, kTab>;
     constexpr int kStore = kMode == 2 ? kNoStore : kPred;
     constexpr uint32_t kStamps = 13;
     __shared__ uint32_t s_dg[kMode == 3 ? G::kWaves * kStamps : 1];
@@ -93,12 +97,11 @@
     };
     constexpr int R = G::kWinRounds, F = G::kFlushRounds;
     __shared__ __attribute__((aligned(16))) uint8_t smem[G::kLdsBytes];
-    uint16_t* s_lo = reinterpret_cast<uint16_t*>(smem + kT8Bytes);
+    uint16_t* s_lo = reinterpret_cast<uint16_t*>(smem);
     uint32_t* s_lut = reinterpret_cast<uint32_t*>(smem + G::kLutOff);
     uint32_t* s_ctr = reinterpret_cast<uint32_t*>(smem + G::kCtrOff);
     uint32_t* s_huge = s_ctr + 16;
     const uint32_t tid = threadIdx.x, lane = tid & 63u, wv = tid >> 6;
-    constexpr int kTab = HPK_LUT3 ? 3 : 2;
     const uint32_t BA = (uint32_t)((uint64_t)a.n * blockIdx.x / gridDim.x);
     const uint32_t BB = (uint32_t)((uint64_t)a.n * (blockIdx.x + 1) / gridDim.x);
     static_assert(G::kBlock == 1024, "the dense check's two offsets rounds");
@@ -119,8 +122,8 @@
     }
     for (uint32_t t = tid; t < kLoBytes / 16; t += G::kBlock)
         reinterpret_cast<uint4*>(s_lo)[t] = reinterpret_cast<const uint4*>(a.lo)[t];
-    for (uint32_t t = tid; t < HPK_LUT_SIZE * 4 / 16; t += G::kBlock)
-        reinterpret_cast<uint4*>(s_lut)[t] = reinterpret_cast<const uint4*>(kTab == 3 ? a.lut3 : a.lut2)[t];
+    for (uint32_t t = tid; t < (uint32_t)G::kLutBytes / 16; t += G::kBlock)
+        reinterpret_cast<uint4*>(s_lut)[t] = reinterpret_cast<const uint4*>(kTab == 4 ? a.lut13 : kTab == 3 ? a.lut3 : a.lut2)[t];
     if (tid < 16) s_ctr[tid] = tid == 7 && kGuided ? min(G::kWaves * c0, BB - BA) : 0u;
     if (kMode == 3)
         for (uint32_t t = tid; t < (uint32_t)G::kWaves * kStamps; t += G::kBlock) s_dg[t] = 0;
@@ -240,7 +243,7 @@
         const uint32_t obase = (uint32_t)(G::kWaveOff + wv * G::kWaveBytes + kWinB);
         const uint32_t* const wl32 = reinterpret_cast<const uint32_t*>(smem);
         uint8_t* const ol8 = smem;
-        const uint32_t dmy = obase + (uint32_t)G::kImg + lane * 4u;
+        const uint32_t dmy = (uint32_t)G::kDummyOff + lane * 4u;
         bool given = false;
         auto claim = [&](uint32_t& ca, uint32_t& ce) {
             if (!kGuided) {
@@ -622,7 +625,7 @@
             stamp(5);
             uint32_t Lend = 0;
             if (kMode != 1) {
-                bool body = L.Eb - L.X >= kBodyMin;
+                bool body = L.Eb - L.X >= body_min<kTab>();
                 uint32_t aX = L.X, aO = L.o, aSt = L.st;
                 bool aAct = L.act, onA = true;
                 for (;;) {
@@ -651,7 +654,7 @@
                             aAct = L.act;
                             load(L, e2, t2);
                             onA = false;
-                            body = L.Eb - L.X >= kBodyMin;
+                            body = L.Eb - L.X >= body_min<kTab>();
                         }
                         if (!__any(body)) break;
                     }
@@ -678,8 +681,8 @@
                         tail12_look<kStore, kTab>(TL, s_lut, ol8, dmy);
                         tail12_look<kStore, kTab>(TN, s_lut, ol8, dmy);
                     }
-                    L.more &= tail12_end(TL, L);
-                    N.more &= tail12_end(TN, N);
+                    L.more &= tail12_end<kTab>(TL, L);
+                    N.more &= tail12_end<kTab>(TN, N);
                 }
                 while (__any(L.more | N.more)) {
                     if (L.more) lit12_step<kStore, true, kTab, true>(L, wl32, s_lut, s_lo, ol8, dmy);
```

Result: faster. 1230 (median of 6 runs) (+7.8%).
